# AI4Science-WestlakeU/wdno

Hardware: AMD Instinct MI355X
Metric: diffusion train steps/sec, 2D smoke U-Net (8 samples per GPU per step) (higher is better)
Workload: dtype f32

## Files before the change

include/wdno_hip.h:

```cpp
#ifndef WDNO_HIP_H
#define WDNO_HIP_H
#include <stdint.h>
#include <stddef.h>

#ifdef __cplusplus
extern "C" {
#endif

typedef void* wdno_stream_t;

enum { WDNO_OK = 0, WDNO_EINVAL = -1, WDNO_ELAUNCH = -2, WDNO_EUNSUPPORTED = -3, WDNO_EWORKSPACE = -4 };

#define WDNO_AMAX_SLOTS 64
#define WDNO_AMAX_STRIDE 16
#define WDNO_AMAX_FLOATS (WDNO_AMAX_SLOTS * WDNO_AMAX_STRIDE)
const char* wdno_strerror(int code);
int wdno_version(void);
const char* wdno_last_hip_error(void);
int wdno_set_debug(int mode);

typedef struct {
  int nd;
  int mode;
  int L;
  int n_img;
  int in_dims[3];
  int out_dims[3];
  int64_t cs_img, cs_band, cs0, cs1;
} wdno_dwt_desc;
size_t wdno_dwt_ws_bytes(const wdno_dwt_desc* d);
int wdno_dwt_fwd(const float* x, float* coef, const wdno_dwt_desc* d, const float* filters_host, void* ws, size_t ws_bytes, wdno_stream_t s);
int wdno_dwt_inv(const float* coef, float* x, const wdno_dwt_desc* d, const float* filters_host, void* ws, size_t ws_bytes, wdno_stream_t s);
int wdno_dwt_fwd_adjoint(const float* dcoef, float* dx, const wdno_dwt_desc* d, const float* filters_host, void* ws, size_t ws_bytes, wdno_stream_t s);
int wdno_dwt_inv_adjoint(const float* dx, float* dcoef, const wdno_dwt_desc* d, const float* filters_host, void* ws, size_t ws_bytes, wdno_stream_t s);
int wdno_dwt_fwd_packed(const float* x, float* state, const wdno_dwt_desc* d, const float* filters_host, int img_inner, int64_t cs_outer, int row_w,
                        const float* rescaler, wdno_stream_t s);
int wdno_upsample_coef(const float* in, float* out, int64_t outer, int a, int mid, int b, int c, int fa, int fb, int fc, wdno_stream_t s);
int wdno_pack_smoke_state(const float* coef, int64_t coef_sim_stride, const float* init_coef, int64_t init_sim_stride, const float* smokeout,
                          int64_t so_sim_stride, const int64_t* idx, const float* rescaler, float* state, int64_t B, int F, int nt, int nx,
                          int pad_t, int pad_x, wdno_stream_t s);
int wdno_pack_smoke_fields(const float* coef, int64_t coef_sim_stride, const float* rho0, int64_t rho0_sim_stride, const float* curve,
                           int64_t curve_sim_stride, const float* dec_lo_host, const float* dec_hi_host, int L, const float* rescaler,
                           float* state, int64_t B, int F, int nt, int nx, int pad_t, int pad_x, int H0, int W0, int T0, wdno_stream_t s);

int wdno_nc_to_cl(const float* src, float* dst, int64_t N, int C, int64_t S, int Cp, wdno_stream_t s);
int wdno_cl_to_nc(const float* src, float* dst, int64_t N, int C, int64_t S, int Cp, wdno_stream_t s);
int wdno_concat2_cl_planes(const float* a, int Ca, const float* b, int Cb, const float* rec_a, const float* rec_b, void* hi, void* lo,
                           float* scale_out, int64_t P, wdno_stream_t s);
int wdno_concat2_cl(const float* a, int Ca, const float* b, int Cb, float* out, int64_t P, wdno_stream_t s);
int wdno_concat2_cl_amax(const float* a, int Ca, const float* b, int Cb, float* out, float* amax_rec, int64_t P, wdno_stream_t s);
int wdno_split2_cl(const float* in, float* a, int Ca, float* b, int Cb, int64_t P, wdno_stream_t s);
int wdno_upsample2x_cl_fwd(const float* in, float* out, int64_t N, int H, int W, int C, wdno_stream_t s);
int wdno_upsample2x_cl_bwd(const float* dout, float* din, int64_t N, int H, int W, int C, wdno_stream_t s);

typedef struct {
  int N, D, H, W, C;
  int OD, OH, OW, K;
  int kd, kh, kw;
  int sd, sh, sw;
  int pd, ph, pw;
  int YD, YH, YW;
  int osd, osh, osw, ood, ooh, oow;
} wdno_conv_geom;
int wdno_conv_fwd(const float* x, const float* wp, const float* bias, const float* residual, float* y,
                  const wdno_conv_geom* g, wdno_stream_t s);
int wdno_amax(const float* x, int64_t n, float* amax_zeroed, wdno_stream_t s);
int wdno_amax_record(const float* x, int64_t n, float* rec_zeroed, wdno_stream_t s);
int wdno_split_f16(const float* x, const float* amax_rec, void* hi, void* lo, float* scale_out, int64_t rows, int C, int C8, wdno_stream_t s);
size_t wdno_split_colsum_ws_bytes(int64_t rows, int C8);
int wdno_split_f16_colsum(const float* x, const float* amax_rec, void* hi, void* lo, float* scale_out, float* colsum_out,
                          void* ws, size_t ws_bytes, int64_t rows, int C, int C8, wdno_stream_t s);
int wdno_pack_split_weight(const float* w, const float* amax, void* hi, void* lo, float* scale_out, int K, int C, int kd, int kh, int kw,
                           int A, int B, int mode, wdno_stream_t s);
typedef struct { const void* x; int64_t n; void* out; } wdno_amax_item;
typedef struct {
  const void* w; const void* amax; void* hi; void* lo; void* scale_out;
  int K, C, kd, kh, kw, A, B, mode;
} wdno_wsplit_item;
int wdno_amax_multi(const void* table, int n_items, int blocks_per_item, wdno_stream_t s);
int wdno_pack_split_weight_multi(const void* table, int n_items, int blocks_per_item, wdno_stream_t s);
int wdno_conv_fwd_f16x3(const void* xh, const void* xl, const float* sx, const void* wph, const void* wpl, const float* sw,
                        const float* bias, const float* residual, float* y, const wdno_conv_geom* g, wdno_stream_t s);
int wdno_conv_fwd_f16x3_amax(const void* xh, const void* xl, const float* sx, const void* wph, const void* wpl, const float* sw,
                             const float* bias, const float* residual, float* y, float* amax_rec, const wdno_conv_geom* g,
                             wdno_stream_t s);
typedef struct { int channels, d0, h0, w0; } wdno_zero_box;
int wdno_conv_fwd_f16x3_zbox(const void* xh, const void* xl, const float* sx, const void* wph, const void* wpl, const float* sw,
                             const float* bias, const float* residual, float* y, float* amax_rec, const wdno_conv_geom* g,
                             const wdno_zero_box* zb, wdno_stream_t s);
int wdno_conv_fwd_bf16_ex(const void* x16, const void* wp16, const float* bias, const float* residual, void* y, int y_bf16, float* amax_rec,
                          const wdno_conv_geom* g, const wdno_zero_box* zb, wdno_stream_t s);
int wdno_conv_fwd_f16x3_ws(const void* xh, const void* xl, const float* sx, const void* wph, const void* wpl, const float* sw,
                           const float* bias, const float* residual, float* y, float* amax_rec, const wdno_conv_geom* g,
                           void* ws, size_t ws_bytes, wdno_stream_t s);
size_t wdno_conv_fwd_split_ws_bytes(const wdno_conv_geom* g);
size_t wdno_conv_wgrad_f16x3_ws_bytes(const wdno_conv_geom* g);
int wdno_conv_pixel_table(void* table, const wdno_conv_geom* g, wdno_stream_t s);
int wdno_conv_wgrad_f16x3(const void* xh, const void* xl, const float* sx, const void* dyh, const void* dyl, const float* sdy,
                          const void* pixel_table, float* dwp, void* ws, size_t ws_bytes, const wdno_conv_geom* g, wdno_stream_t s);
int wdno_conv_wgrad_f16x3_param(const void* xh, const void* xl, const float* sx, const void* dyh, const void* dyl, const float* sdy,
                                const void* pixel_table, float* dw, int Kn, int Cn, void* ws, size_t ws_bytes,
                                const wdno_conv_geom* g, wdno_stream_t s);
#define WDNO_WGRAD_REDUCE_MAX 40
typedef struct wdno_wgrad_reduce_item {
  const float* ws; float* dw;
  int n, splits;
  int K8, C8, kw, ntap, Kn, Cn;
  int tiled;
  int reserved;
} wdno_wgrad_reduce_item;
int wdno_conv_wgrad_partials(const void* xh, const void* xl, const float* sx, const void* dyh, const void* dyl, const float* sdy,
                             const void* pixel_table, float* dw, int Kn, int Cn, void* ws, size_t ws_bytes,
                             const wdno_conv_geom* g, wdno_wgrad_reduce_item* item, wdno_stream_t s);
int wdno_wgrad_reduce_multi(const wdno_wgrad_reduce_item* items, int n_items, wdno_stream_t s);
size_t wdno_conv_wgrad_ws_bytes(const wdno_conv_geom* g);
int wdno_conv_wgrad(const float* x, const float* dy, float* dwp, void* ws, size_t ws_bytes,
                    const wdno_conv_geom* g, wdno_stream_t s);
#define WDNO_ROWS_SUM_MAX 64
typedef struct wdno_rows_sum_item {
  const void* part; float* out;
  int rows, stride, col0, ncols;
  int is_double, reserved;
} wdno_rows_sum_item;
int wdno_rows_sum_multi(const wdno_rows_sum_item* items, int n_items, wdno_stream_t s);
size_t wdno_colsum_ws_bytes(int64_t P, int C);
int wdno_colsum(const float* in, float* out, int64_t P, int C, void* ws, size_t ws_bytes, wdno_stream_t s);

int wdno_cast_bf16(const float* x, void* out16, int64_t rows, int C, int C8, wdno_stream_t s);
int wdno_cast_bf16_colsum(const float* x, void* out16, float* colsum_out, void* ws, size_t ws_bytes, int64_t rows, int C, int C8, wdno_stream_t s);
int wdno_conv_fwd_bf16(const void* x16, const void* wp16, const float* bias, const float* residual, float* y, float* amax_rec,
                       const wdno_conv_geom* g, wdno_stream_t s);
int wdno_conv_wgrad_bf16_param(const void* x16, const void* dy16, const void* pixel_table, float* dw, int Kn, int Cn, void* ws,
                               size_t ws_bytes, const wdno_conv_geom* g, wdno_stream_t s);

size_t wdno_groupnorm_ws_bytes(int64_t N, int64_t S, int C, int G);
size_t wdno_groupnorm_stats_floats(int64_t N, int C, int G);
int wdno_groupnorm_act_fwd(const float* x, const float* gamma, const float* beta, const float* ss, float* y,
                           float* stats, int64_t N, int64_t S, int C, int G, float eps, int silu,
                           void* ws, size_t ws_bytes, wdno_stream_t s);
int wdno_groupnorm_act_fwd_amax(const float* x, const float* gamma, const float* beta, const float* ss, float* y,
                                float* stats, float* amax_rec, int64_t N, int64_t S, int C, int G, float eps, int silu,
                                void* ws, size_t ws_bytes, wdno_stream_t s);
int wdno_groupnorm_act_bwd(const float* x, const float* dy, const float* gamma, const float* beta, const float* ss,
                           const float* stats, float* dx, float* dgb_partial, float* dss,
                           int64_t N, int64_t S, int C, int G, int silu, void* ws, size_t ws_bytes, wdno_stream_t s);
int wdno_groupnorm_act_bwd_amax(const float* x, const float* dy, const float* gamma, const float* beta, const float* ss,
                                const float* stats, float* dx, float* dgb_partial, float* dss, float* amax_rec,
                                int64_t N, int64_t S, int C, int G, int silu, void* ws, size_t ws_bytes, wdno_stream_t s);
size_t wdno_groupnorm_bwd_planes_ws_bytes(int64_t N, int64_t S, int C, int G);
size_t wdno_groupnorm_fwd_planes_ws_bytes(int64_t N, int64_t S, int C, int G);
int wdno_groupnorm_act_fwd_planes(const float* x, const float* gamma, const float* beta, const float* ss, void* y_hi, void* y_lo,
                                  float* y_scale, float* stats, float* bound_rec, int64_t N, int64_t S, int C, int G, float eps, int silu,
                                  void* ws, size_t ws_bytes, wdno_stream_t s);
int wdno_groupnorm_act_add_fwd_planes(const float* x, const float* gamma, const float* beta, const float* ss, const float* residual,
                                      const float* res_rec, float* y, void* y_hi, void* y_lo, float* y_scale, float* stats,
                                      float* bound_rec, float* y_amax_rec, int64_t N, int64_t S, int C, int G, float eps, int silu,
                                      void* ws, size_t ws_bytes, wdno_stream_t s);
int wdno_groupnorm_act_bwd_planes(const float* x, const float* dy, const float* gamma, const float* beta, const float* ss,
                                  const float* stats, void* dx_hi, void* dx_lo, float* dx_scale, float* dx_colsum,
                                  float* dgb_partial, float* dgb_sum, float* dss, float* bound_rec, int64_t N, int64_t S, int C, int G, int silu,
                                  void* ws, size_t ws_bytes, wdno_stream_t s);
int wdno_groupnorm_bwd_planes_tail(int64_t N, int64_t S, int C, int G, size_t* csp_offset, int* rows);
int wdno_groupnorm_act_fwd_amax_t(const void* x, int x_bf16, const float* gamma, const float* beta, const float* ss, float* y,
                                  float* stats, float* amax_rec, int64_t N, int64_t S, int C, int G, float eps, int silu,
                                  void* ws, size_t ws_bytes, wdno_stream_t s);
int wdno_groupnorm_act_fwd_planes_t(const void* x, int x_bf16, const float* gamma, const float* beta, const float* ss, void* y_hi, void* y_lo,
                                    float* y_scale, float* stats, float* bound_rec, int64_t N, int64_t S, int C, int G, float eps,
                                    int silu, void* ws, size_t ws_bytes, wdno_stream_t s);
int wdno_groupnorm_act_add_fwd_planes_t(const void* x, int x_bf16, const float* gamma, const float* beta, const float* ss, const float* residual,
                                        const float* res_rec, float* y, void* y_hi, void* y_lo, float* y_scale, float* stats,
                                        float* bound_rec, float* y_amax_rec, int64_t N, int64_t S, int C, int G, float eps, int silu,
                                        void* ws, size_t ws_bytes, wdno_stream_t s);
int wdno_groupnorm_act_bwd_planes_t(const void* x, int x_bf16, const void* dy, int dy_bf16, const float* gamma, const float* beta, const float* ss,
                                    const float* stats, void* dx_hi, void* dx_lo, float* dx_scale, float* dx_colsum,
                                    float* dgb_partial, float* dgb_sum, float* dss, float* bound_rec, int64_t N, int64_t S, int C, int G, int silu,
                                    void* ws, size_t ws_bytes, wdno_stream_t s);
int wdno_layernorm_fwd(const float* x, const float* g, float* y, int64_t P, int C, float eps, wdno_stream_t s);
int wdno_layernorm_fwd_amax(const float* x, const float* g, float* y, float* amax_rec, int64_t P, int C, float eps, wdno_stream_t s);
int wdno_layernorm_fwd_planes(const float* x, const float* g, void* y_hi, void* y_lo, float* y_scale, int64_t P, int C, float eps,
                              wdno_stream_t s);
size_t wdno_layernorm_bwd_ws_bytes(int64_t P, int C);
int wdno_layernorm_bwd(const float* x, const float* g, const float* dy, float* dx, float* dg, int64_t P, int C,
                       float eps, void* ws, size_t ws_bytes, wdno_stream_t s);
int wdno_layernorm_bwd_add(const float* x, const float* g, const float* dy, const float* add_to, float* dx, float* dg, int64_t P, int C,
                           float eps, void* ws, size_t ws_bytes, wdno_stream_t s);
int wdno_layernorm_bwd_add_amax(const float* x, const float* g, const float* dy, const float* add_to, float* dx, float* dg, float* amax_rec,
                                int64_t P, int C, float eps, void* ws, size_t ws_bytes, wdno_stream_t s);

typedef struct {
  int n_uo, n_ui, n_tok, heads;
  int64_t so, si, st;
} wdno_attn_desc;
int wdno_attn_fwd(const float* qkv, const float* rot_cos, const float* rot_sin, const float* bias, float* out,
                  const wdno_attn_desc* d, float scale, wdno_stream_t s);
size_t wdno_attn_bwd_ws_bytes(const wdno_attn_desc* d);
int wdno_attn_bwd(const float* qkv, const float* rot_cos, const float* rot_sin, const float* bias, const float* out,
                  const float* dout, float* dqkv, float* dbias, const wdno_attn_desc* d, float scale, void* ws, size_t ws_bytes,
                  wdno_stream_t s);
int wdno_attn_fwd_amax(const float* qkv, const float* rot_cos, const float* rot_sin, const float* bias, float* out, float* amax_rec,
                       const wdno_attn_desc* d, float scale, wdno_stream_t s);
int wdno_attn_bwd_amax(const float* qkv, const float* rot_cos, const float* rot_sin, const float* bias, const float* out,
                       const float* dout, float* dqkv, float* dbias, float* amax_rec, const wdno_attn_desc* d, float scale,
                       void* ws, size_t ws_bytes, wdno_stream_t s);
int wdno_attn_bwd_planes(const float* qkv, const float* rot_cos, const float* rot_sin, const float* bias, const float* out,
                         const float* dout, void* dqkv_hi, void* dqkv_lo, float* dqkv_scale, float* dbias,
                         const float* rec_qkv, const float* rec_dout, const wdno_attn_desc* d, float scale, void* ws, size_t ws_bytes,
                         wdno_stream_t s);
int wdno_attn_fwd_planes(const float* qkv, const float* rot_cos, const float* rot_sin, const float* bias, float* out, void* out_hi,
                         void* out_lo, float* out_scale, float* amax_rec, const float* rec_qkv, const wdno_attn_desc* d, float scale,
                         wdno_stream_t s);
size_t wdno_linattn_ws_bytes(int64_t units, int heads);
int wdno_linattn_fwd(const float* qkv, float* out, float* kstats , float* ctx ,
                     int64_t units, int n_tok, int heads, float scale, wdno_stream_t s);
int wdno_linattn_bwd(const float* qkv, const float* dout, const float* kstats, const float* ctx, float* dqkv,
                     void* ws, size_t ws_bytes, int64_t units, int n_tok, int heads, float scale, wdno_stream_t s);
int wdno_linattn_fwd_amax(const float* qkv, float* out, float* kstats, float* ctx, float* amax_rec, int64_t units, int n_tok, int heads,
                          float scale, wdno_stream_t s);
int wdno_linattn_bwd_amax(const float* qkv, const float* dout, const float* kstats, const float* ctx, float* dqkv, float* amax_rec,
                          void* ws, size_t ws_bytes, int64_t units, int n_tok, int heads, float scale, wdno_stream_t s);
int wdno_linattn_bwd_planes(const float* qkv, const float* dout, const float* kstats, const float* ctx, void* dqkv_hi, void* dqkv_lo,
                            float* dqkv_scale, const float* rec_qkv, const float* rec_dout, float* rec_dctx, void* ws, size_t ws_bytes,
                            int64_t units, int n_tok, int heads, float scale, wdno_stream_t s);
int wdno_linattn_fwd_planes(const float* qkv, void* out_hi, void* out_lo, float* out_scale, float* kstats, float* ctx,
                            const float* rec_qkv, int64_t units, int n_tok, int heads, float scale, wdno_stream_t s);

int wdno_tattn_fused_takes(int C, int n_tok, int heads);
int wdno_tattn_fused_fwd(const float* x, const float* gamma, float eps, const void* wq_hi, const void* wq_lo, const float* wq_scale,
                         const void* wo_hi, const void* wo_lo, const float* wo_scale, const float* rot_cos, const float* rot_sin,
                         const float* bias, float* y, float* amax_rec, float* qkv_out, float* rec_v,
                         int64_t n_batch, int n_tok, int64_t hw, int C, int heads, float scale, wdno_stream_t s);
size_t wdno_tattn_fused_bwd_ws_bytes(void);
int wdno_tattn_fused_bwd_grads(void);
int wdno_tattn_fused_bwd(const float* x, const float* dy, const float* gamma, float eps, const void* wq_hi, const void* wq_lo,
                         const float* wq_scale, const void* wo_hi, const void* wo_lo, const float* wo_scale, const float* rot_cos,
                         const float* rot_sin, const float* bias, const float* rec_dy, const float* rec_v, float* dx, float* amax_rec,
                         float* grads, void* ws, size_t ws_bytes,
                         int64_t n_batch, int n_tok, int64_t hw, int C, int heads, float scale, wdno_stream_t s);

int wdno_lattn_fused_takes(int C, int heads, int n_tok);
size_t wdno_lattn_fused_ws_bytes(int64_t units, int n_tok);
int wdno_lattn_fused_fwd(const float* x, const float* gamma, float eps, const void* wq_hi, const void* wq_lo, const float* wq_scale,
                         const void* wo_hi, const void* wo_lo, const float* wo_scale, const float* bias_out, float* y, float* amax_rec,
                         float* ctx_out, float* kstat_out, void* ws, size_t ws_bytes, int64_t units, int n_tok, int C, int heads, float scale,
                         wdno_stream_t s);

int wdno_lattn_fused_bwd_grads(void);
size_t wdno_lattn_fused_bwd_ws_bytes(int64_t units, int n_tok);
int wdno_lattn_fused_bwd(const float* x, const float* dy, const float* gamma, float eps, const void* wq_hi, const void* wq_lo,
                         const float* wq_scale, const void* wot_hi, const void* wot_lo, const float* wot_scale, const float* ctx,
                         const float* kstat, const float* rec_dy, float* dx, float* amax_rec, float* grads, void* ws, size_t ws_bytes,
                         int64_t units, int n_tok, int C, int heads, float scale, wdno_stream_t s);

int wdno_relpos_bias_fwd(const float* w, const int64_t* bucket, float* out, int n, int heads, wdno_stream_t s);
int wdno_relpos_bias_bwd(const float* dbias, const int64_t* bucket, float* dw, int n, int heads, int num_buckets, wdno_stream_t s);

int wdno_linear_rows_fwd(const float* x, int x_stride, const float* w, int w_stride, const float* bias, float* y, int P, int C, int K,
                         int Kp, wdno_stream_t s);
int wdno_linear_rows_wgrad(const float* x, int x_stride, const float* dy, int dy_stride, float* dw, float* db, int P, int C, int K,
                           wdno_stream_t s);

typedef struct wdno_linear_item {
  const void* w;
  const void* bias;
  int K, k_start;
} wdno_linear_item;
int wdno_linear_multi_fwd(const void* table, int n_items, int F, const float* x, float* y, int P, int C, wdno_stream_t s);
int wdno_linear_multi_wgrad(const void* table, int n_items, int F, const float* x, const float* dy, float* dw, float* db, int P, int C,
                            wdno_stream_t s);
size_t wdno_linear_multi_dgrad_ws_bytes(int F, int P, int C);
int wdno_linear_multi_dgrad(const void* table, int n_items, int F, const float* dy, float* dx, int P, int C, void* ws, size_t ws_bytes,
                            wdno_stream_t s);

int wdno_act_fwd(const float* x, float* y, int64_t n, int act, wdno_stream_t s);
int wdno_act_bwd(const float* x, const float* dy, float* dx, int64_t n, int act, wdno_stream_t s);
int wdno_add(const float* a, const float* b, float* out, int64_t n, wdno_stream_t s);
int wdno_add_amax(const float* a, const float* b, float* out, float* amax_rec, int64_t n, wdno_stream_t s);
int wdno_sinusoidal_emb(const int64_t* t, const float* freqs, float* out, int B, int dim, wdno_stream_t s);

typedef struct {
  int tree;
  int B, F, C, H, W;
  int cT, cH, cW;
  int cond_pad, cond_a, cond_b, cond_c, cond_low;
  int u_rows, uT_rows;
} wdno_cond_desc;
int wdno_q_sample_cond(const float* x0, const float* noise, const int64_t* t, const float* sqrt_ac, const float* sqrt_1mac,
                       float* x_out, float* target_out, const wdno_cond_desc* c, wdno_stream_t s);
int wdno_apply_cond(float* x, const float* src, const wdno_cond_desc* c, wdno_stream_t s);
int wdno_weighted_mse(const float* out, const float* target, const float* wc, const float* wb, float inv_count,
                      float* loss, float* grad, int64_t B, int64_t per_sample, int C, int64_t inner,
                      void* ws, size_t ws_bytes, wdno_stream_t s);
size_t wdno_weighted_mse_ws_bytes(int64_t n);
int wdno_weighted_mse_bwd(const float* out, const float* target, const float* wc, const float* wb, float inv_count,
                          const float* gscale, float* grad, int64_t B, int64_t per_sample, int C, int64_t inner, wdno_stream_t s);
int wdno_p_sample_update(const float* x, const float* eps, const float* noise, const int64_t* t,
                         const float* sqrt_recip_ac, const float* sqrt_recipm1_ac, const float* pm1, const float* pm2,
                         const float* plogvar, float* x_next, float* x_start, int64_t B, int64_t per_sample, int clamp, wdno_stream_t s);
int wdno_ddim_update(const float* x, const float* eps, const float* noise, const int64_t* t,
                     const float* sqrt_recip_ac, const float* sqrt_recipm1_ac, float sqrt_an, float c, float sigma,
                     float* x_next, float* x_start, int64_t B, int64_t per_sample, wdno_stream_t s);
int wdno_ddim_update_dev(const float* x, const float* eps, const float* noise, const int64_t* t,
                         const float* sqrt_recip_ac, const float* sqrt_recipm1_ac, const float* coef_dev,
                         float* x_next, float* x_start, int64_t B, int64_t per_sample, wdno_stream_t s);

size_t wdno_sumsq_ws_bytes(int64_t n);
int wdno_sumsq(const float* g, int64_t n, float* out, void* ws, size_t ws_bytes, wdno_stream_t s);
int wdno_adam_clip_step(float* p, const float* g, float* m, float* v, int64_t n, const float* sumsq, float max_norm,
                        float grad_scale, float lr, float beta1, float beta2, float eps, int step, wdno_stream_t s);
typedef struct { const void* src; void* dst; int64_t n; } wdno_copy_item;
int wdno_gather_items(const void* table, int n_items, int blocks_per_item, wdno_stream_t s);
int wdno_ema_update(float* ema, const float* p, int64_t n, float beta, wdno_stream_t s);

typedef struct {
  int N, s, nx0, nt_f, nxf;
  int steps, record_time, f_time, num_t, sub_s, out_cols;
  int waves, points;
  float c, d, dm, dt;
} wdno_burgers_desc;
int wdno_burgers_solve(const float* u0, const float* f, float* out, const wdno_burgers_desc* d, wdno_stream_t s);

typedef struct {
  int N, s, t;
  int steps, record_time, f_time, num_t;
  int st, sx, f_rows, cols;
  int waves, points, clamp;
  float c, d, dm, dt, alpha;
} wdno_burgers_generate_desc;
int wdno_burgers_generate(const float* u0, const float* ax, const float* tt, float* u_rec, float* f_rec,
                          const wdno_burgers_generate_desc* d, wdno_stream_t s);

typedef struct {
  int B, C, H, W;
  int sample_stride, chan_stride, row_stride;
  int h, w, n_t, n_x;
  int L, mode;
  int ntile, tw, lds_bytes;
  int num_timesteps;
  int condition_f, clip_x0;
  float wu, wf;
} wdno_burgers_guidance_desc;
int wdno_burgers_guidance(const float* x_t, const float* in, const int64_t* t, const float* c1, const float* c2, const float* s_table,
                          const float* rescaler, const float* target, float* out, const wdno_burgers_guidance_desc* d, const float* filt,
                          wdno_stream_t s);

typedef struct {
  int B, nt, nx, time_interval, space_interval;
  int num_t, max_iter, n_out, threads;
  float accuracy;
} wdno_smoke_solve_desc;
int wdno_smoke_solve(const float* init_density, const float* c1, const float* c2, const float* init_velocity, const float* fluid_ext,
                     const float* active_ext, const float* velocity_mask, const float* buckets, const int* frame_slot, float* density,
                     float* zero_density, float* velocity, double* ratio, float* ws, const wdno_smoke_solve_desc* d, wdno_stream_t s);

typedef struct {
  int B, scenelength, record_scale, stride;
  int max_iter, threads, noise_mode;
  float accuracy;
  unsigned long long seed;
} wdno_smoke_generate_desc;
int wdno_smoke_generate(const int* scene_i, const float* scene_v, const long long* scene_index, const double* noise,
                        const float* init_velocity, const float* fluid_ext, const float* active_ext, const float* velocity_mask,
                        const float* buckets, float* density, float* velocity, float* control, double* smoke, float* ws,
                        const wdno_smoke_generate_desc* d, wdno_stream_t s);
int wdno_smoke_noise(const long long* scene_index, const int* frame, const int* is_kick, const float* kick_v, int n,
                     unsigned long long seed, float* out, wdno_stream_t s);

#ifdef __cplusplus
}
#endif
#endif
```

wdno_amd/_lib.py:

```python
import contextlib
import ctypes as C
import os

import torch

HERE = os.path.dirname(os.path.abspath(__file__))
LIB_PATH = os.path.join(HERE, 'libwdno_hip.so')

P = C.c_void_p
I = C.c_int
L = C.c_int64
F = C.c_float
Z = C.c_size_t


class DwtDesc(C.Structure):
    _fields_ = [('nd', I), ('mode', I), ('L', I), ('n_img', I), ('in_dims', I * 3), ('out_dims', I * 3),
                ('cs_img', L), ('cs_band', L), ('cs0', L), ('cs1', L)]


class ConvGeom(C.Structure):
    _fields_ = [(k, I) for k in ('N', 'D', 'H', 'W', 'C', 'OD', 'OH', 'OW', 'K', 'kd', 'kh', 'kw', 'sd', 'sh', 'sw',
                                 'pd', 'ph', 'pw', 'YD', 'YH', 'YW', 'osd', 'osh', 'osw', 'ood', 'ooh', 'oow')]


class AttnDesc(C.Structure):
    _fields_ = [('n_uo', I), ('n_ui', I), ('n_tok', I), ('heads', I), ('so', L), ('si', L), ('st', L)]


class CondDesc(C.Structure):
    _fields_ = [(k, I) for k in ('tree', 'B', 'F', 'C', 'H', 'W', 'cT', 'cH', 'cW', 'cond_pad', 'cond_a', 'cond_b',
                                 'cond_c', 'cond_low', 'u_rows', 'uT_rows')]


class WgradReduceItem(C.Structure):
    _fields_ = [('ws', C.c_void_p), ('dw', C.c_void_p), ('n', I), ('splits', I), ('K8', I), ('C8', I), ('kw', I), ('ntap', I), ('Kn', I), ('Cn', I),
                ('tiled', I), ('reserved', I)]


class RowsSumItem(C.Structure):
    _fields_ = [('part', C.c_void_p), ('out', C.c_void_p), ('rows', I), ('stride', I), ('col0', I), ('ncols', I), ('is_double', I), ('reserved', I)]


class BurgersDesc(C.Structure):
    _fields_ = [(k, I) for k in ('N', 's', 'nx0', 'nt_f', 'nxf', 'steps', 'record_time', 'f_time', 'num_t', 'sub_s', 'out_cols', 'waves',
                                 'points')] + [(k, F) for k in ('c', 'd', 'dm', 'dt')]


class BurgersGenerateDesc(C.Structure):
    _fields_ = [(k, I) for k in ('N', 's', 't', 'steps', 'record_time', 'f_time', 'num_t', 'st', 'sx', 'f_rows', 'cols', 'waves', 'points',
                                 'clamp')] + [(k, F) for k in ('c', 'd', 'dm', 'dt', 'alpha')]


class BurgersGuidanceDesc(C.Structure):
    _fields_ = [(k, I) for k in ('B', 'C', 'H', 'W', 'sample_stride', 'chan_stride', 'row_stride', 'h', 'w', 'n_t', 'n_x', 'L', 'mode', 'ntile',
                                 'tw', 'lds_bytes', 'num_timesteps', 'condition_f', 'clip_x0')] + [(k, F) for k in ('wu', 'wf')]


class SmokeSolveDesc(C.Structure):
    _fields_ = [(k, I) for k in ('B', 'nt', 'nx', 'time_interval', 'space_interval', 'num_t', 'max_iter', 'n_out', 'threads')] + [('accuracy', F)]


class SmokeGenerateDesc(C.Structure):
    _fields_ = [(k, I) for k in ('B', 'scenelength', 'record_scale', 'stride', 'max_iter', 'threads', 'noise_mode')] + [('accuracy', F), ('seed', C.c_uint64)]


PD, PG, PA, PC = C.POINTER(DwtDesc), C.POINTER(ConvGeom), C.POINTER(AttnDesc), C.POINTER(CondDesc)
PF = C.POINTER(C.c_float)

PROTOTYPES = {
    'wdno_strerror': (C.c_char_p, [I]),
    'wdno_version': (I, []),
    'wdno_last_hip_error': (C.c_char_p, []),
    'wdno_set_debug': (I, [I]),
    'wdno_dwt_ws_bytes': (Z, [PD]),
    'wdno_dwt_fwd': (I, [P, P, PD, PF, P, Z, P]),
    'wdno_dwt_fwd_packed': (I, [P, P, PD, PF, I, L, I, P, P]),
    'wdno_dwt_inv': (I, [P, P, PD, PF, P, Z, P]),
    'wdno_dwt_fwd_adjoint': (I, [P, P, PD, PF, P, Z, P]),
    'wdno_dwt_inv_adjoint': (I, [P, P, PD, PF, P, Z, P]),
    'wdno_upsample_coef': (I, [P, P, L, I, I, I, I, I, I, I, P]),
    'wdno_pack_smoke_state': (I, [P, L, P, L, P, L, P, P, P, L, I, I, I, I, I, P]),
    'wdno_pack_smoke_fields': (I, [P, L, P, L, P, L, PF, PF, I, P, P, L, I, I, I, I, I, I, I, I, P]),
    'wdno_nc_to_cl': (I, [P, P, L, I, L, I, P]),
    'wdno_cl_to_nc': (I, [P, P, L, I, L, I, P]),
    'wdno_concat2_cl': (I, [P, I, P, I, P, L, P]),
    'wdno_concat2_cl_planes': (I, [P, I, P, I, P, P, P, P, P, L, P]),
    'wdno_concat2_cl_amax': (I, [P, I, P, I, P, P, L, P]),
    'wdno_split2_cl': (I, [P, P, I, P, I, L, P]),
    'wdno_upsample2x_cl_fwd': (I, [P, P, L, I, I, I, P]),
    'wdno_upsample2x_cl_bwd': (I, [P, P, L, I, I, I, P]),
    'wdno_conv_fwd': (I, [P, P, P, P, P, PG, P]),
    'wdno_amax': (I, [P, L, P, P]),
    'wdno_amax_record': (I, [P, L, P, P]),
    'wdno_split_f16': (I, [P, P, P, P, P, L, I, I, P]),
    'wdno_split_colsum_ws_bytes': (Z, [L, I]),
    'wdno_split_f16_colsum': (I, [P, P, P, P, P, P, P, Z, L, I, I, P]),
    'wdno_pack_split_weight': (I, [P, P, P, P, P, I, I, I, I, I, I, I, I, P]),
    'wdno_amax_multi': (I, [P, I, I, P]),
    'wdno_pack_split_weight_multi': (I, [P, I, I, P]),
    'wdno_conv_fwd_f16x3': (I, [P, P, P, P, P, P, P, P, P, PG, P]),
    'wdno_conv_fwd_f16x3_amax': (I, [P, P, P, P, P, P, P, P, P, P, PG, P]),
    'wdno_conv_fwd_f16x3_ws': (I, [P, P, P, P, P, P, P, P, P, P, PG, P, Z, P]),
    'wdno_conv_fwd_split_ws_bytes': (Z, [PG]),
    'wdno_conv_wgrad_f16x3_ws_bytes': (Z, [PG]),
    'wdno_conv_pixel_table': (I, [P, PG, P]),
    'wdno_conv_wgrad_f16x3': (I, [P, P, P, P, P, P, P, P, P, Z, PG, P]),
    'wdno_conv_wgrad_f16x3_param': (I, [P, P, P, P, P, P, P, P, I, I, P, Z, PG, P]),
    'wdno_conv_wgrad_partials': (I, [P, P, P, P, P, P, P, P, I, I, P, Z, PG, P, P]),
    'wdno_wgrad_reduce_multi': (I, [P, I, P]),
    'wdno_rows_sum_multi': (I, [P, I, P]),
    'wdno_cast_bf16': (I, [P, P, L, I, I, P]),
    'wdno_cast_bf16_colsum': (I, [P, P, P, P, Z, L, I, I, P]),
    'wdno_conv_fwd_bf16': (I, [P, P, P, P, P, P, PG, P]),
    'wdno_conv_fwd_f16x3_zbox': (I, [P, P, P, P, P, P, P, P, P, P, PG, P, P]),
    'wdno_conv_fwd_bf16_ex': (I, [P, P, P, P, P, I, P, PG, P, P]),
    'wdno_conv_wgrad_bf16_param': (I, [P, P, P, P, I, I, P, Z, PG, P]),
    'wdno_conv_wgrad_ws_bytes': (Z, [PG]),
    'wdno_conv_wgrad': (I, [P, P, P, P, Z, PG, P]),
    'wdno_colsum_ws_bytes': (Z, [L, I]),
    'wdno_colsum': (I, [P, P, L, I, P, Z, P]),
    'wdno_groupnorm_ws_bytes': (Z, [L, L, I, I]),
    'wdno_groupnorm_stats_floats': (Z, [L, I, I]),
    'wdno_groupnorm_act_fwd': (I, [P, P, P, P, P, P, L, L, I, I, F, I, P, Z, P]),
    'wdno_groupnorm_act_fwd_amax': (I, [P, P, P, P, P, P, P, L, L, I, I, F, I, P, Z, P]),
    'wdno_groupnorm_act_bwd': (I, [P, P, P, P, P, P, P, P, P, L, L, I, I, I, P, Z, P]),
    'wdno_groupnorm_act_bwd_amax': (I, [P, P, P, P, P, P, P, P, P, P, L, L, I, I, I, P, Z, P]),
    'wdno_groupnorm_bwd_planes_ws_bytes': (Z, [L, L, I, I]),
    'wdno_groupnorm_bwd_planes_tail': (I, [L, L, I, I, C.POINTER(Z), C.POINTER(I)]),
    'wdno_groupnorm_fwd_planes_ws_bytes': (Z, [L, L, I, I]),
    'wdno_groupnorm_act_fwd_planes': (I, [P, P, P, P, P, P, P, P, P, L, L, I, I, F, I, P, Z, P]),
    'wdno_groupnorm_act_add_fwd_planes': (I, [P, P, P, P, P, P, P, P, P, P, P, P, P, L, L, I, I, F, I, P, Z, P]),
    'wdno_layernorm_fwd_planes': (I, [P, P, P, P, P, L, I, F, P]),
    'wdno_groupnorm_act_bwd_planes': (I, [P, P, P, P, P, P, P, P, P, P, P, P, P, P, L, L, I, I, I, P, Z, P]),
    'wdno_groupnorm_act_fwd_amax_t': (I, [P, I, P, P, P, P, P, P, L, L, I, I, F, I, P, Z, P]),
    'wdno_groupnorm_act_fwd_planes_t': (I, [P, I, P, P, P, P, P, P, P, P, L, L, I, I, F, I, P, Z, P]),
    'wdno_groupnorm_act_add_fwd_planes_t': (I, [P, I, P, P, P, P, P, P, P, P, P, P, P, P, L, L, I, I, F, I, P, Z, P]),
    'wdno_groupnorm_act_bwd_planes_t': (I, [P, I, P, I, P, P, P, P, P, P, P, P, P, P, P, P, L, L, I, I, I, P, Z, P]),
    'wdno_layernorm_fwd': (I, [P, P, P, L, I, F, P]),
    'wdno_layernorm_fwd_amax': (I, [P, P, P, P, L, I, F, P]),
    'wdno_layernorm_bwd_ws_bytes': (Z, [L, I]),
    'wdno_layernorm_bwd': (I, [P, P, P, P, P, L, I, F, P, Z, P]),
    'wdno_layernorm_bwd_add': (I, [P, P, P, P, P, P, L, I, F, P, Z, P]),
    'wdno_layernorm_bwd_add_amax': (I, [P, P, P, P, P, P, P, L, I, F, P, Z, P]),
    'wdno_attn_fwd': (I, [P, P, P, P, P, PA, F, P]),
    'wdno_attn_bwd_ws_bytes': (Z, [PA]),
    'wdno_attn_bwd': (I, [P, P, P, P, P, P, P, P, PA, F, P, Z, P]),
    'wdno_attn_fwd_amax': (I, [P, P, P, P, P, P, PA, F, P]),
    'wdno_attn_bwd_amax': (I, [P, P, P, P, P, P, P, P, P, PA, F, P, Z, P]),
    'wdno_attn_fwd_planes': (I, [P, P, P, P, P, P, P, P, P, P, PA, F, P]),
    'wdno_linattn_fwd_planes': (I, [P, P, P, P, P, P, P, L, I, I, F, P]),
    'wdno_attn_bwd_planes': (I, [P, P, P, P, P, P, P, P, P, P, P, P, PA, F, P, Z, P]),
    'wdno_tattn_fused_takes': (I, [I, I, I]),
    'wdno_tattn_fused_fwd': (I, [P, P, F, P, P, P, P, P, P, P, P, P, P, P, P, P, L, I, L, I, I, F, P]),
    'wdno_lattn_fused_takes': (I, [I, I, I]),
    'wdno_lattn_fused_ws_bytes': (Z, [L, I]),
    'wdno_lattn_fused_fwd': (I, [P, P, F, P, P, P, P, P, P, P, P, P, P, P, P, Z, L, I, I, I, F, P]),
    'wdno_lattn_fused_bwd_grads': (I, []),
    'wdno_lattn_fused_bwd_ws_bytes': (Z, [L, I]),
    'wdno_lattn_fused_bwd': (I, [P, P, P, F, P, P, P, P, P, P, P, P, P, P, P, P, P, Z, L, I, I, I, F, P]),
    'wdno_tattn_fused_bwd_ws_bytes': (Z, []),
    'wdno_tattn_fused_bwd_grads': (I, []),
    'wdno_tattn_fused_bwd': (I, [P, P, P, F, P, P, P, P, P, P, P, P, P, P, P, P, P, P, P, Z, L, I, L, I, I, F, P]),
    'wdno_linattn_ws_bytes': (Z, [L, I]),
    'wdno_linattn_fwd': (I, [P, P, P, P, L, I, I, F, P]),
    'wdno_linattn_bwd': (I, [P, P, P, P, P, P, Z, L, I, I, F, P]),
    'wdno_linattn_fwd_amax': (I, [P, P, P, P, P, L, I, I, F, P]),
    'wdno_linattn_bwd_amax': (I, [P, P, P, P, P, P, P, Z, L, I, I, F, P]),
    'wdno_linattn_bwd_planes': (I, [P, P, P, P, P, P, P, P, P, P, P, Z, L, I, I, F, P]),
    'wdno_act_fwd': (I, [P, P, L, I, P]),
    'wdno_act_bwd': (I, [P, P, P, L, I, P]),
    'wdno_linear_rows_fwd': (I, [P, I, P, I, P, P, I, I, I, I, P]),
    'wdno_linear_rows_wgrad': (I, [P, I, P, I, P, P, I, I, I, P]),
    'wdno_linear_multi_fwd': (I, [P, I, I, P, P, I, I, P]),
    'wdno_linear_multi_wgrad': (I, [P, I, I, P, P, P, P, I, I, P]),
    'wdno_linear_multi_dgrad_ws_bytes': (Z, [I, I, I]),
    'wdno_linear_multi_dgrad': (I, [P, I, I, P, P, I, I, P, Z, P]),
    'wdno_add': (I, [P, P, P, L, P]),
    'wdno_add_amax': (I, [P, P, P, P, L, P]),
    'wdno_sinusoidal_emb': (I, [P, P, P, I, I, P]),
    'wdno_q_sample_cond': (I, [P, P, P, P, P, P, P, PC, P]),
    'wdno_apply_cond': (I, [P, P, PC, P]),
    'wdno_weighted_mse_ws_bytes': (Z, [L]),
    'wdno_weighted_mse': (I, [P, P, P, P, F, P, P, L, L, I, L, P, Z, P]),
    'wdno_weighted_mse_bwd': (I, [P, P, P, P, F, P, P, L, L, I, L, P]),
    'wdno_p_sample_update': (I, [P, P, P, P, P, P, P, P, P, P, P, L, L, I, P]),
    'wdno_ddim_update': (I, [P, P, P, P, P, P, F, F, F, P, P, L, L, P]),
    'wdno_ddim_update_dev': (I, [P, P, P, P, P, P, P, P, P, L, L, P]),
    'wdno_sumsq_ws_bytes': (Z, [L]),
    'wdno_sumsq': (I, [P, L, P, P, Z, P]),
    'wdno_adam_clip_step': (I, [P, P, P, P, L, P, F, F, F, F, F, F, I, P]),
    'wdno_ema_update': (I, [P, P, L, F, P]),
    'wdno_gather_items': (I, [P, I, I, P]),
    'wdno_relpos_bias_fwd': (I, [P, P, P, I, I, P]),
    'wdno_relpos_bias_bwd': (I, [P, P, P, I, I, I, P]),
    'wdno_burgers_solve': (I, [P, P, P, C.POINTER(BurgersDesc), P]),
    'wdno_burgers_generate': (I, [P, P, P, P, P, C.POINTER(BurgersGenerateDesc), P]),
    'wdno_burgers_guidance': (I, [P, P, P, P, P, P, P, P, P, C.POINTER(BurgersGuidanceDesc), PF, P]),
    'wdno_smoke_solve': (I, [P, P, P, P, P, P, P, P, P, P, P, P, P, P, C.POINTER(SmokeSolveDesc), P]),
    'wdno_smoke_generate': (I, [P, P, P, P, P, P, P, P, P, P, P, P, P, P, C.POINTER(SmokeGenerateDesc), P]),
    'wdno_smoke_noise': (I, [P, P, P, P, I, C.c_uint64, P, P]),
}

_lib = None


def load():
    global _lib
    if _lib is not None:
        return _lib
    if not os.path.exists(LIB_PATH):
        raise RuntimeError(f'{LIB_PATH} is missing: run `python -c "import __graft_entry__ as g; g.build()"` '
                           '(there is no CPU / eager fallback for the wdno_amd hot path)')
    lib = C.CDLL(LIB_PATH)
    for name, (res, args) in PROTOTYPES.items():
        fn = getattr(lib, name)
        fn.restype = res
        fn.argtypes = args
    _lib = lib
    if os.environ.get('WDNO_DEBUG'):
        try:
            check(lib.wdno_set_debug(int(os.environ['WDNO_DEBUG'])), f"WDNO_DEBUG={os.environ['WDNO_DEBUG']}")
        except RuntimeError:
            _lib = None
            raise
    return lib


def check(code, what):
    if code != 0:
        lib = load()
        msg = lib.wdno_strerror(code).decode()
        hip = lib.wdno_last_hip_error().decode() if code == -2 else ''
        raise RuntimeError(f'{what} failed: {msg} ({code}) {hip}')


@contextlib.contextmanager
def debug_mode(mode):
    lib = load()
    check(lib.wdno_set_debug(mode), f'wdno_set_debug({mode})')
    try:
        yield
    finally:
        lib.wdno_set_debug(0)
```

wdno_amd/csrc/common.h:

```cpp
#pragma once
#include <hip/hip_runtime.h>
#include <stdint.h>
#include "../../include/wdno_hip.h"

extern thread_local hipError_t wdno_tls_last_hip_error;

static inline int wdno_check_launch() {
  hipError_t e = hipGetLastError();
  if (e != hipSuccess) {
    wdno_tls_last_hip_error = e;
    return WDNO_ELAUNCH;
  }
  return WDNO_OK;
}

#define WDNO_REQUIRE(cond)            \
  do {                                \
    if (!(cond)) return WDNO_EINVAL;  \
  } while (0)

static inline hipStream_t as_stream(wdno_stream_t s) { return reinterpret_cast<hipStream_t>(s); }

int wdno_num_cus();

static inline int64_t cdiv64(int64_t a, int64_t b) { return (a + b - 1) / b; }
static inline int cdiv(int a, int b) { return (a + b - 1) / b; }

static inline int stream_grid(int64_t work_items, int block) {
  int64_t g = cdiv64(work_items, block);
  if (g > 2048) g = 2048;
  if (g < 1) g = 1;
  return (int)g;
}

#ifdef __HIPCC__
__device__ __forceinline__ float wave_sum(float v) {
#pragma unroll
  for (int o = 32; o > 0; o >>= 1) v += __shfl_xor(v, o, 64);
  return v;
}
__device__ __forceinline__ double wave_sum_d(double v) {
#pragma unroll
  for (int o = 32; o > 0; o >>= 1) v += __shfl_xor(v, o, 64);
  return v;
}
__device__ __forceinline__ float wave_max(float v) {
#pragma unroll
  for (int o = 32; o > 0; o >>= 1) v = fmaxf(v, __shfl_xor(v, o, 64));
  return v;
}
__device__ __forceinline__ void amax_record_emit(float m, float* __restrict__ rec, unsigned block_linear) {
  __shared__ float amax_red[4];
  m = wave_max(m);
  if ((threadIdx.x & 63) == 0) amax_red[(threadIdx.x >> 6) & 3] = m;
  __syncthreads();
  if (threadIdx.x == 0) {
    m = fmaxf(fmaxf(amax_red[0], amax_red[1]), fmaxf(amax_red[2], amax_red[3]));
    atomicMax(reinterpret_cast<unsigned*>(rec) + (block_linear & (WDNO_AMAX_SLOTS - 1)) * WDNO_AMAX_STRIDE, __float_as_uint(m));
  }
}
__device__ __forceinline__ void wave_amax_emit(float am, float* rec, int wave_linear) {
  am = wave_max(am);
  if ((threadIdx.x & 63) == 0)
    atomicMax(reinterpret_cast<unsigned*>(rec) + (wave_linear & (WDNO_AMAX_SLOTS - 1)) * WDNO_AMAX_STRIDE, __float_as_uint(am));
}
__device__ __forceinline__ float amax_record_read(const float* __restrict__ rec) {
  return wave_max(rec[(threadIdx.x & (WDNO_AMAX_SLOTS - 1)) * WDNO_AMAX_STRIDE]);
}
__device__ __forceinline__ unsigned short bf16_rne(float v) {
  unsigned u = __float_as_uint(v);
  if ((u & 0x7fffffffu) > 0x7f800000u) return (unsigned short)((u >> 16) | 0x40u);
  return (unsigned short)((u + 0x7fffu + ((u >> 16) & 1u)) >> 16);
}
__device__ __forceinline__ uint2 bf16x4_pack(float4 v) {
  return make_uint2((unsigned)bf16_rne(v.x) | ((unsigned)bf16_rne(v.y) << 16), (unsigned)bf16_rne(v.z) | ((unsigned)bf16_rne(v.w) << 16));
}
__device__ __forceinline__ void plane_pack(float v, float s, bool lp, _Float16& h, _Float16& l) {
  if (lp) { const unsigned short b = bf16_rne(v); h = __builtin_bit_cast(_Float16, b); l = (_Float16)0.f; return; }
  const float t = v * s;
  h = (_Float16)t;
  l = (_Float16)(t - (float)h);
}
__device__ __forceinline__ float scale_from_amax(float amax) {
  if (!(amax > 0.f) || !isfinite(amax)) return 1.0f;
  int e = ilogbf(amax);
  return ldexpf(1.0f, 14 - e);
}
__device__ __forceinline__ float amax4(float m, float4 v) {
  return fmaxf(fmaxf(m, fmaxf(fabsf(v.x), fabsf(v.y))), fmaxf(fabsf(v.z), fabsf(v.w)));
}
template <int W>
__device__ __forceinline__ float group_sum(float v) {
#pragma unroll
  for (int o = W / 2; o > 0; o >>= 1) v += __shfl_xor(v, o, 64);
  return v;
}
template <int W>
__device__ __forceinline__ float group_max(float v) {
#pragma unroll
  for (int o = W / 2; o > 0; o >>= 1) v = fmaxf(v, __shfl_xor(v, o, 64));
  return v;
}
#define PRS_GROUPS 32
#define PRS_THREADS (32 * PRS_GROUPS)
template <typename T>
__device__ __forceinline__ void partial_rows_sum_body(const T* __restrict__ part, float* __restrict__ out, int nb, int C, int bx, int stride = 0) {
  __shared__ double red[PRS_GROUPS][33];
  const int tx = threadIdx.x & 31, ty = threadIdx.x >> 5;
  const int c = bx * 32 + tx;
  if (stride == 0) stride = C;
  double acc = 0.0;
  if (c < C) {
    double a0 = 0.0, a1 = 0.0, a2 = 0.0, a3 = 0.0;
    int b = ty;
    for (; b + 3 * PRS_GROUPS < nb; b += 4 * PRS_GROUPS) {
      a0 += (double)part[(int64_t)b * stride + c];
      a1 += (double)part[(int64_t)(b + PRS_GROUPS) * stride + c];
      a2 += (double)part[(int64_t)(b + 2 * PRS_GROUPS) * stride + c];
      a3 += (double)part[(int64_t)(b + 3 * PRS_GROUPS) * stride + c];
    }
    for (; b < nb; b += PRS_GROUPS) a0 += (double)part[(int64_t)b * stride + c];
    acc = (a0 + a1) + (a2 + a3);
  }
  red[ty][tx] = acc;
  __syncthreads();
  if (ty == 0 && c < C) {
    double a[4] = {0.0, 0.0, 0.0, 0.0};
#pragma unroll
    for (int g = 0; g < PRS_GROUPS; ++g) a[g & 3] += red[g][tx];
    out[c] = (float)((a[0] + a[1]) + (a[2] + a[3]));
  }
}
template <typename T>
__global__ __launch_bounds__(PRS_THREADS) void partial_rows_sum_kernel(const T* __restrict__ part, float* __restrict__ out, int nb, int C) {
  partial_rows_sum_body<T>(part, out, nb, C, (int)blockIdx.x);
}

__device__ __forceinline__ float silu_f(float z) { return z / (1.0f + expf(-z)); }
__device__ __forceinline__ float silu_grad_f(float z) {
  float sg = 1.0f / (1.0f + expf(-z));
  return sg * (1.0f + z * (1.0f - sg));
}
#endif
```

wdno_amd/csrc/norm.hip:

```cpp
#include "common.h"
#include <type_traits>

#define GN_MAXC 1024

struct gn_bf16 {};
template <typename T> struct gn_ld;
template <> struct gn_ld<float> {
  static __device__ __forceinline__ float4 ld4(const void* p, int64_t e) { return *reinterpret_cast<const float4*>(static_cast<const float*>(p) + e); }
};
template <> struct gn_ld<gn_bf16> {
  static __device__ __forceinline__ float4 ld4(const void* p, int64_t e) {
    const uint2 u = *reinterpret_cast<const uint2*>(static_cast<const unsigned short*>(p) + e);
    return make_float4(__uint_as_float(u.x << 16), __uint_as_float(u.x & 0xffff0000u), __uint_as_float(u.y << 16), __uint_as_float(u.y & 0xffff0000u));
  }
};
template <typename T> __device__ __forceinline__ void gn_ld8(const void* p, int64_t e, float (&v)[8]) {
  const float4 a = gn_ld<T>::ld4(p, e), b = gn_ld<T>::ld4(p, e + 4);
  v[0] = a.x; v[1] = a.y; v[2] = a.z; v[3] = a.w; v[4] = b.x; v[5] = b.y; v[6] = b.z; v[7] = b.w;
}

static inline int pow2ceil(int v) { int p = 1; while (p < v) p <<= 1; return p; }
static inline int gn_chunks(int64_t S, int64_t N, int C) {
  int64_t c = cdiv64(S, 64);
  if (c > 64) c = 64;
  if (c < 1) c = 1;
  int txp = pow2ceil(C >> 2);
  if (txp > 256) txp = 256;
  const int nty = 256 / (txp < 1 ? 1 : txp);
  const int64_t cap = N > 0 && 512 / N > 64 ? 512 / N : 64;
  while (c < cap && N * c < 256 && S / (2 * c) >= 4 * nty) c *= 2;
  return (int)c;
}

template <int MODE, typename XT = float, typename DT = float>
__global__ __launch_bounds__(256) void gn_partial_kernel(const void* __restrict__ x, const void* __restrict__ dy,
                                                          const float* __restrict__ cb , const float* __restrict__ gb ,
                                                          double* __restrict__ part, int64_t S, int C, int cg, int G, int txp,
                                                          int64_t rows_per_chunk, int silu, float* __restrict__ mx = nullptr) {
  __shared__ double red[256 * 8];
  __shared__ float redm[8];
  float m0[4] = {0.f, 0.f, 0.f, 0.f}, m1[4] = {0.f, 0.f, 0.f, 0.f};
  const int n = blockIdx.y, chunk = blockIdx.x, nchunk = gridDim.x;
  const int C4 = C >> 2;
  const int tx = threadIdx.x & (txp - 1), ty = threadIdx.x / txp, nty = 256 / txp;
  const int64_t r0 = (int64_t)chunk * rows_per_chunk;
  int64_t r1 = r0 + rows_per_chunk;
  if (r1 > S) r1 = S;
  double s0[4] = {0, 0, 0, 0}, s1[4] = {0, 0, 0, 0};
  if (tx < C4) {
    float ca[4], cbb[4], mean[4], rstd[4];
    if (MODE == 1) {
#pragma unroll
      for (int j = 0; j < 4; ++j) {
        int c = tx * 4 + j;
        ca[j] = cb[((int64_t)n * C + c) * 4 + 0];
        cbb[j] = cb[((int64_t)n * C + c) * 4 + 1];
        int g = c / cg;
        mean[j] = gb[((int64_t)n * G + g) * 4 + 0];
        rstd[j] = gb[((int64_t)n * G + g) * 4 + 1];
      }
    }
    const int64_t e0 = ((int64_t)n * S) * C + tx * 4;
    constexpr int RIF = std::is_same<XT, gn_bf16>::value ? 8 : 4;
    for (int64_t rb = r0 + ty; rb < r1; rb += RIF * nty) {
      float4 vv[RIF], dd[RIF];
#pragma unroll
      for (int u = 0; u < RIF; ++u) {
        const int64_t r = rb + u * nty;
        const bool ok = r < r1;
        vv[u] = ok ? gn_ld<XT>::ld4(x, e0 + r * C) : make_float4(0.f, 0.f, 0.f, 0.f);
        if (MODE == 1) dd[u] = ok ? gn_ld<DT>::ld4(dy, e0 + r * C) : make_float4(0.f, 0.f, 0.f, 0.f);
      }
#pragma unroll
      for (int u = 0; u < RIF; ++u) {
        if (rb + u * nty >= r1) break;
        const float4 v = vv[u];
        float xv[4] = {v.x, v.y, v.z, v.w};
        if (MODE == 0) {
#pragma unroll
          for (int j = 0; j < 4; ++j) { s0[j] += (double)xv[j]; s1[j] += (double)xv[j] * (double)xv[j]; m0[j] = fmaxf(m0[j], fabsf(xv[j])); }
        } else {
          const float4 d = dd[u];
          float dv[4] = {d.x, d.y, d.z, d.w};
#pragma unroll
          for (int j = 0; j < 4; ++j) {
            float dz = dv[j];
            if (silu) dz *= silu_grad_f(ca[j] * xv[j] + cbb[j]);
            float xh = (xv[j] - mean[j]) * rstd[j];
            s0[j] += (double)dz;
            s1[j] += (double)dz * (double)xh;
            m0[j] = fmaxf(m0[j], fabsf(dz)); m1[j] = fmaxf(m1[j], fabsf(xh));
          }
        }
      }
    }
  }
#pragma unroll
  for (int j = 0; j < 4; ++j) { red[(ty * txp + tx) * 8 + j] = s0[j]; red[(ty * txp + tx) * 8 + 4 + j] = s1[j]; }
  __syncthreads();
  if (ty == 0 && tx < C4) {
    for (int t = 1; t < nty; ++t)
#pragma unroll
      for (int j = 0; j < 4; ++j) { s0[j] += red[(t * txp + tx) * 8 + j]; s1[j] += red[(t * txp + tx) * 8 + 4 + j]; }
    double* o = part + (((int64_t)n * nchunk + chunk) * C + tx * 4) * 2;
#pragma unroll
    for (int j = 0; j < 4; ++j) { o[j * 2] = s0[j]; o[j * 2 + 1] = s1[j]; }
  }
  if (mx) {
    float a = fmaxf(fmaxf(m0[0], m0[1]), fmaxf(m0[2], m0[3])), b = fmaxf(fmaxf(m1[0], m1[1]), fmaxf(m1[2], m1[3]));
    a = wave_max(a); b = wave_max(b);
    if ((threadIdx.x & 63) == 0) { redm[(threadIdx.x >> 6) * 2] = a; redm[(threadIdx.x >> 6) * 2 + 1] = b; }
    __syncthreads();
    if (threadIdx.x == 0) {
      float* o = mx + ((int64_t)n * nchunk + chunk) * 2;
      o[0] = fmaxf(fmaxf(redm[0], redm[2]), fmaxf(redm[4], redm[6]));
      o[1] = fmaxf(fmaxf(redm[1], redm[3]), fmaxf(redm[5], redm[7]));
    }
  }
}

__device__ __forceinline__ void gn_chunk_totals(const double* __restrict__ part, int n, int nchunk, int Call, double* sa, double* sb, int cb0 = 0, int cn = -1) {
  const int C = cn < 0 ? Call : cn;
  part += cb0 * 2;
  const int nsub = C <= 128 ? 256 / C : 1;
  for (int idx = threadIdx.x; idx < C * nsub; idx += 256) {
    const int q = idx / C, c = idx - q * C;
    const int k1 = (q + 1) * nchunk / nsub;
    int k = q * nchunk / nsub;
    double a0 = 0, b0 = 0, a1 = 0, b1 = 0;
    for (; k + 7 < k1; k += 8) {
      const double* q0 = part + (((int64_t)n * nchunk + k) * Call + c) * 2;
      double va[8], vb[8];
#pragma unroll
      for (int u = 0; u < 8; ++u) { va[u] = q0[(int64_t)u * Call * 2]; vb[u] = q0[(int64_t)u * Call * 2 + 1]; }
#pragma unroll
      for (int u = 0; u < 8; u += 2) { a0 += va[u]; b0 += vb[u]; a1 += va[u + 1]; b1 += vb[u + 1]; }
    }
    for (; k + 1 < k1; k += 2) {
      const double* q0 = part + (((int64_t)n * nchunk + k) * Call + c) * 2;
      const double* q1 = q0 + (int64_t)Call * 2;
      a0 += q0[0]; b0 += q0[1]; a1 += q1[0]; b1 += q1[1];
    }
    if (k < k1) {
      const double* q0 = part + (((int64_t)n * nchunk + k) * Call + c) * 2;
      a0 += q0[0]; b0 += q0[1];
    }
    sa[idx] = a0 + a1; sb[idx] = b0 + b1;
  }
  __syncthreads();
  if (nsub > 1) {
    const int c = threadIdx.x;
    double a = 0, b = 0;
    if (c < C)
      for (int q = 0; q < nsub; ++q) { a += sa[q * C + c]; b += sb[q * C + c]; }
    __syncthreads();
    if (c < C) { sa[c] = a; sb[c] = b; }
    __syncthreads();
  }
}

__global__ __launch_bounds__(256) void gn_finalize_kernel(const double* __restrict__ part, const float* __restrict__ stats_in,
                                                           const float* __restrict__ gamma, const float* __restrict__ beta,
                                                           const float* __restrict__ ss, float* __restrict__ stats_out,
                                                           float* __restrict__ cb, float* __restrict__ gb, int64_t S, int C, int G,
                                                           int nchunk, float eps, const float* __restrict__ mx = nullptr,
                                                           float* __restrict__ bound_rec = nullptr) {
  __shared__ double chs[GN_MAXC], chq[GN_MAXC];
  __shared__ float gmean[GN_MAXC], grstd[GN_MAXC];
  const int n = blockIdx.x, cg = C / G;
  const int gps = (G + (int)gridDim.y - 1) / (int)gridDim.y, gs0 = (int)blockIdx.y * gps, gs1 = min(G, gs0 + gps);
  if (gs0 >= gs1) return;
  const int cs0 = gs0 * cg, csn = (gs1 - gs0) * cg;
  gamma += cs0; beta += cs0;
  if (ss) ss += cs0;
  cb += (int64_t)cs0 * 4; gb += (int64_t)gs0 * 4;
  if (stats_out) stats_out += (int64_t)gs0 * 2;
  if (stats_in) stats_in += (int64_t)gs0 * 2;
  const int Call = C, Gall = G;
  C = csn; G = gs1 - gs0;
  if (part) {
    gn_chunk_totals(part, n, nchunk, Call, chs, chq, cs0, csn);
    if (cg > 64) {
      __shared__ double ra[256], rb[256];
      for (int g = 0; g < G; ++g) {
        double a = 0, b = 0;
        for (int c = g * cg + threadIdx.x; c < (g + 1) * cg; c += 256) { a += chs[c]; b += chq[c]; }
        ra[threadIdx.x] = a; rb[threadIdx.x] = b;
        __syncthreads();
        for (int o = 128; o > 0; o >>= 1) {
          if (threadIdx.x < o) { ra[threadIdx.x] += ra[threadIdx.x + o]; rb[threadIdx.x] += rb[threadIdx.x + o]; }
          __syncthreads();
        }
        if (threadIdx.x == 0) { chs[g * cg] = ra[0]; chq[g * cg] = rb[0]; }
        __syncthreads();
      }
    }
    for (int g = threadIdx.x; g < G; g += 256) {
      double a = 0, b = 0;
      if (cg > 64) { a = chs[g * cg]; b = chq[g * cg]; }
      else for (int c = g * cg; c < (g + 1) * cg; ++c) { a += chs[c]; b += chq[c]; }
      double m = (double)cg * (double)S;
      double mean = a / m;
      double var = b / m - mean * mean;
      if (var < 0) var = 0;
      float rstd = (float)(1.0 / sqrt(var + (double)eps));
      gmean[g] = (float)mean; grstd[g] = rstd;
      stats_out[((int64_t)n * Gall + g) * 2 + 0] = (float)mean;
      stats_out[((int64_t)n * Gall + g) * 2 + 1] = rstd;
    }
  } else {
    for (int g = threadIdx.x; g < G; g += 256) {
      gmean[g] = stats_in[((int64_t)n * Gall + g) * 2 + 0];
      grstd[g] = stats_in[((int64_t)n * Gall + g) * 2 + 1];
    }
  }
  __syncthreads();
  for (int g = threadIdx.x; g < G; g += 256) {
    float* o = gb + ((int64_t)n * Gall + g) * 4;
    o[0] = gmean[g]; o[1] = grstd[g]; o[2] = 0.f; o[3] = 0.f;
  }
  float ma = 0.f, mb = 0.f;
  for (int c = threadIdx.x; c < C; c += 256) {
    int g = c / cg;
    float sc1 = ss ? ss[(int64_t)n * 2 * Call + c] + 1.0f : 1.0f;
    float sh = ss ? ss[(int64_t)n * 2 * Call + Call + c] : 0.0f;
    float k1 = grstd[g] * gamma[c];
    float a = k1 * sc1;
    float b = (beta[c] - gmean[g] * k1) * sc1 + sh;
    float* o = cb + ((int64_t)n * Call + c) * 4;
    o[0] = a; o[1] = b; o[2] = a; o[3] = 0.f;
    ma = fmaxf(ma, fabsf(a)); mb = fmaxf(mb, fabsf(b));
  }
  if (bound_rec) {
    float mxx = 0.f;
    for (int k = threadIdx.x; k < nchunk; k += 256) mxx = fmaxf(mxx, mx[((int64_t)n * nchunk + k) * 2]);
    __shared__ float bm[3][4];
    float v[3] = {wave_max(ma), wave_max(mb), wave_max(mxx)};
    if ((threadIdx.x & 63) == 0)
      for (int q = 0; q < 3; ++q) bm[q][threadIdx.x >> 6] = v[q];
    __syncthreads();
    if (threadIdx.x == 0) {
      float t[3];
      for (int q = 0; q < 3; ++q) t[q] = fmaxf(fmaxf(bm[q][0], bm[q][1]), fmaxf(bm[q][2], bm[q][3]));
      atomicMax(reinterpret_cast<unsigned*>(bound_rec) + (n & (WDNO_AMAX_SLOTS - 1)) * WDNO_AMAX_STRIDE, __float_as_uint(t[0] * t[2] + t[1]));
    }
  }
}

template <typename XT = float>
__global__ __launch_bounds__(256) void gn_apply_kernel(const void* __restrict__ x, const float* __restrict__ cb, float* __restrict__ y,
                                                        int64_t S, int C, int silu, float* __restrict__ amax_rec) {
  const int n = blockIdx.y;
  const int C4 = C >> 2;
  const int64_t total4 = S * C4;
  const int64_t xe = (int64_t)n * S * C;
  float4* yp = reinterpret_cast<float4*>(y + (int64_t)n * S * C);
  const float4* cbp = reinterpret_cast<const float4*>(cb + (int64_t)n * C * 4);
  const int64_t stride = (int64_t)gridDim.x * 256;
  float am = 0.f;
  for (int64_t i = (int64_t)blockIdx.x * 256 + threadIdx.x; i < total4; i += stride) {
    int c4 = (int)(i % C4);
    float4 v = gn_ld<XT>::ld4(x, xe + i * 4);
    float4 k0 = cbp[c4 * 4 + 0], k1 = cbp[c4 * 4 + 1], k2 = cbp[c4 * 4 + 2], k3 = cbp[c4 * 4 + 3];
    float4 o;
    o.x = k0.x * v.x + k0.y; o.y = k1.x * v.y + k1.y; o.z = k2.x * v.z + k2.y; o.w = k3.x * v.w + k3.y;
    if (silu) { o.x = silu_f(o.x); o.y = silu_f(o.y); o.z = silu_f(o.z); o.w = silu_f(o.w); }
    yp[i] = o;
    am = amax4(am, o);
  }
  if (amax_rec) amax_record_emit(am, amax_rec, blockIdx.y * gridDim.x + blockIdx.x);
}

__global__ __launch_bounds__(256) void gn_bwd_finalize_kernel(const double* __restrict__ part, const float* __restrict__ gamma,
                                                               const float* __restrict__ beta, const float* __restrict__ ss,
                                                               float* __restrict__ gb, float* __restrict__ dgb, float* __restrict__ dss,
                                                               int64_t S, int C, int G, int nchunk, const float* __restrict__ cb = nullptr,
                                                               const float* __restrict__ mx = nullptr, float* __restrict__ bound_rec = nullptr) {
  __shared__ double chA[GN_MAXC], chB[GN_MAXC];
  const int n = blockIdx.x, cg = C / G;
  const int gps = (G + (int)gridDim.y - 1) / (int)gridDim.y, gs0 = (int)blockIdx.y * gps, gs1 = min(G, gs0 + gps);
  if (gs0 >= gs1) return;
  const int cs0 = gs0 * cg, csn = (gs1 - gs0) * cg;
  gamma += cs0; beta += cs0;
  if (ss) ss += cs0;
  if (dss) dss += cs0;
  dgb += cs0; gb += (int64_t)gs0 * 4;
  if (cb) cb += (int64_t)cs0 * 4;
  const int Call = C, Gall = G;
  C = csn; G = gs1 - gs0;
  gn_chunk_totals(part, n, nchunk, Call, chA, chB, cs0, csn);
  for (int c = threadIdx.x; c < C; c += 256) {
    const double a = chA[c], b = chB[c];
    float sc1 = ss ? ss[(int64_t)n * 2 * Call + c] + 1.0f : 1.0f;
    if (dss) {
      dss[(int64_t)n * 2 * Call + c] = (float)((double)gamma[c] * b + (double)beta[c] * a);
      dss[(int64_t)n * 2 * Call + Call + c] = (float)a;
    }
    dgb[((int64_t)n * 2 + 0) * Call + c] = (float)((double)sc1 * b);
    dgb[((int64_t)n * 2 + 1) * Call + c] = (float)((double)sc1 * a);
    double w = (double)gamma[c] * (double)sc1;
    chA[c] = w * a; chB[c] = w * b;
  }
  __syncthreads();
  if (cg > 64) {
    __shared__ double ra[256], rb[256];
    for (int g = 0; g < G; ++g) {
      double a = 0, b = 0;
      for (int c = g * cg + threadIdx.x; c < (g + 1) * cg; c += 256) { a += chA[c]; b += chB[c]; }
      ra[threadIdx.x] = a; rb[threadIdx.x] = b;
      __syncthreads();
      for (int o = 128; o > 0; o >>= 1) {
        if (threadIdx.x < o) { ra[threadIdx.x] += ra[threadIdx.x + o]; rb[threadIdx.x] += rb[threadIdx.x + o]; }
        __syncthreads();
      }
      if (threadIdx.x == 0) { chA[g * cg] = ra[0]; chB[g * cg] = rb[0]; }
      __syncthreads();
    }
  }
  for (int g = threadIdx.x; g < G; g += 256) {
    double a = 0, b = 0;
    if (cg > 64) { a = chA[g * cg]; b = chB[g * cg]; }
    else for (int c = g * cg; c < (g + 1) * cg; ++c) { a += chA[c]; b += chB[c]; }
    double m = (double)cg * (double)S;
    float* o = gb + ((int64_t)n * Gall + g) * 4;
    float rstd = o[1];
    o[2] = (float)(a / m) * rstd;
    o[3] = (float)(b / m) * rstd;
  }
  if (bound_rec) {
    __syncthreads();
    float mdz = 0.f, mxh = 0.f, mk = 0.f, mz = 0.f, mw = 0.f;
    for (int k = threadIdx.x; k < nchunk; k += 256) {
      mdz = fmaxf(mdz, mx[((int64_t)n * nchunk + k) * 2]); mxh = fmaxf(mxh, mx[((int64_t)n * nchunk + k) * 2 + 1]);
    }
    for (int c = threadIdx.x; c < C; c += 256) mk = fmaxf(mk, fabsf(cb[((int64_t)n * Call + c) * 4 + 2]));
    for (int g = threadIdx.x; g < G; g += 256) {
      mz = fmaxf(mz, fabsf(gb[((int64_t)n * Gall + g) * 4 + 2])); mw = fmaxf(mw, fabsf(gb[((int64_t)n * Gall + g) * 4 + 3]));
    }
    __shared__ float bm[5][4];
    float v[5] = {wave_max(mdz), wave_max(mxh), wave_max(mk), wave_max(mz), wave_max(mw)};
    if ((threadIdx.x & 63) == 0)
      for (int q = 0; q < 5; ++q) bm[q][threadIdx.x >> 6] = v[q];
    __syncthreads();
    if (threadIdx.x == 0) {
      float t[5];
      for (int q = 0; q < 5; ++q) t[q] = fmaxf(fmaxf(bm[q][0], bm[q][1]), fmaxf(bm[q][2], bm[q][3]));
      const float bound = t[2] * t[0] + t[3] + t[1] * t[4];
      atomicMax(reinterpret_cast<unsigned*>(bound_rec) + (n & (WDNO_AMAX_SLOTS - 1)) * WDNO_AMAX_STRIDE, __float_as_uint(bound));
    }
  }
}

__global__ __launch_bounds__(256) void gn_bwd_apply_kernel(const float* __restrict__ x, const float* __restrict__ dy,
                                                            const float* __restrict__ cb, const float* __restrict__ gb,
                                                            float* __restrict__ dx, int64_t S, int C, int cg, int G, int silu,
                                                            float* __restrict__ amax_rec) {
  const int n = blockIdx.y;
  const int C4 = C >> 2;
  const int64_t total4 = S * C4;
  const float4* xp = reinterpret_cast<const float4*>(x + (int64_t)n * S * C);
  const float4* dp = reinterpret_cast<const float4*>(dy + (int64_t)n * S * C);
  float4* op = reinterpret_cast<float4*>(dx + (int64_t)n * S * C);
  const float4* cbp = reinterpret_cast<const float4*>(cb + (int64_t)n * C * 4);
  const float4* gbp = reinterpret_cast<const float4*>(gb + (int64_t)n * G * 4);
  const int64_t stride = (int64_t)gridDim.x * 256;
  float am = 0.f;
  for (int64_t i = (int64_t)blockIdx.x * 256 + threadIdx.x; i < total4; i += stride) {
    int c4 = (int)(i % C4);
    float4 v = xp[i], d = dp[i];
    float xv[4] = {v.x, v.y, v.z, v.w}, dv[4] = {d.x, d.y, d.z, d.w}, o[4];
#pragma unroll
    for (int j = 0; j < 4; ++j) {
      int c = c4 * 4 + j;
      float4 k = cbp[c];
      float4 gq = gbp[c / cg];
      float dz = dv[j];
      if (silu) dz *= silu_grad_f(k.x * xv[j] + k.y);
      float xh = (xv[j] - gq.x) * gq.y;
      o[j] = k.z * dz - gq.z - xh * gq.w;
    }
    op[i] = make_float4(o[0], o[1], o[2], o[3]);
    am = fmaxf(fmaxf(am, fmaxf(fabsf(o[0]), fabsf(o[1]))), fmaxf(fabsf(o[2]), fabsf(o[3])));
  }
  if (amax_rec) amax_record_emit(am, amax_rec, blockIdx.y * gridDim.x + blockIdx.x);
}

typedef _Float16 gn_half8 __attribute__((ext_vector_type(8)));
template <typename XT = float>
__global__ __launch_bounds__(256) void gn_apply_planes_kernel(const void* __restrict__ x, const float* __restrict__ cb,
                                                               _Float16* __restrict__ hi, _Float16* __restrict__ lo,
                                                               float* __restrict__ scale_out, const float* __restrict__ rec,
                                                               int64_t S, int C, int silu) {
  const int n = blockIdx.y;
  const int C8 = C >> 3;
  const int64_t total8 = S * C8;
  const bool single = lo == nullptr;
  const float s = single ? 1.0f : scale_from_amax(amax_record_read(rec));
  if (!single && blockIdx.x == 0 && blockIdx.y == 0 && threadIdx.x == 0) scale_out[0] = s;
  const int64_t xe = (int64_t)n * S * C;
  _Float16* hp = hi + (int64_t)n * S * C;
  _Float16* lp = single ? nullptr : lo + (int64_t)n * S * C;
  const float4* cbp = reinterpret_cast<const float4*>(cb + (int64_t)n * C * 4);
  const int64_t stride = (int64_t)gridDim.x * 256;
  const int c0 = (int)(((int64_t)blockIdx.x * 256 + threadIdx.x) % C8) * 8;
  float ka[8], kb[8];
#pragma unroll
  for (int j = 0; j < 8; ++j) { const float4 k = cbp[c0 + j]; ka[j] = k.x; kb[j] = k.y; }
  for (int64_t i = (int64_t)blockIdx.x * 256 + threadIdx.x; i < total8; i += stride) {
    float xv[8];
    gn_ld8<XT>(x, xe + i * 8, xv);
    gn_half8 h, l;
#pragma unroll
    for (int j = 0; j < 8; ++j) {
      float o = ka[j] * xv[j] + kb[j];
      if (silu) o = silu_f(o);
      _Float16 th, tl;
      plane_pack(o, s, single, th, tl);
      h[j] = th; l[j] = tl;
    }
    *reinterpret_cast<gn_half8*>(hp + i * 8) = h;
    if (!single) *reinterpret_cast<gn_half8*>(lp + i * 8) = l;
  }
}

template <typename XT = float>
__global__ __launch_bounds__(256) void gn_apply_add_planes_kernel(const void* __restrict__ x, const float* __restrict__ cb,
                                                                   const float* __restrict__ res, float* __restrict__ y,
                                                                   _Float16* __restrict__ hi, _Float16* __restrict__ lo,
                                                                   float* __restrict__ scale_out, const float* __restrict__ rec,
                                                                   const float* __restrict__ rec_res, float* __restrict__ amax_out,
                                                                   int64_t S, int C, int silu) {
  const int n = blockIdx.y;
  const int C8 = C >> 3;
  const int64_t total8 = S * C8;
  const bool planes = hi != nullptr;
  const bool single = lo == nullptr;
  const float s = single ? 1.0f : scale_from_amax(amax_record_read(rec) + amax_record_read(rec_res));
  if (!single && blockIdx.x == 0 && blockIdx.y == 0 && threadIdx.x == 0) scale_out[0] = s;
  const int64_t xe = (int64_t)n * S * C;
  const float* rp = res + (int64_t)n * S * C;
  float* yp = y + (int64_t)n * S * C;
  _Float16* hp = planes ? hi + (int64_t)n * S * C : nullptr;
  _Float16* lp = single ? nullptr : lo + (int64_t)n * S * C;
  const float4* cbp = reinterpret_cast<const float4*>(cb + (int64_t)n * C * 4);
  const int64_t stride = (int64_t)gridDim.x * 256;
  const int c0 = (int)(((int64_t)blockIdx.x * 256 + threadIdx.x) % C8) * 8;
  float ka[8], kb[8];
#pragma unroll
  for (int j = 0; j < 8; ++j) { const float4 k = cbp[c0 + j]; ka[j] = k.x; kb[j] = k.y; }
  float am = 0.f;
  for (int64_t i = (int64_t)blockIdx.x * 256 + threadIdx.x; i < total8; i += stride) {
    float xv[8];
    gn_ld8<XT>(x, xe + i * 8, xv);
    const float4 r0 = *reinterpret_cast<const float4*>(rp + i * 8), r1 = *reinterpret_cast<const float4*>(rp + i * 8 + 4);
    const float rv[8] = {r0.x, r0.y, r0.z, r0.w, r1.x, r1.y, r1.z, r1.w};
    float ov[8];
    gn_half8 h, l;
#pragma unroll
    for (int j = 0; j < 8; ++j) {
      float o = ka[j] * xv[j] + kb[j];
      if (silu) o = silu_f(o);
      o += rv[j];
      ov[j] = o;
      am = fmaxf(am, fabsf(o));
      _Float16 th, tl;
      plane_pack(o, s, single, th, tl);
      h[j] = th; l[j] = tl;
    }
    *reinterpret_cast<float4*>(yp + i * 8) = make_float4(ov[0], ov[1], ov[2], ov[3]);
    *reinterpret_cast<float4*>(yp + i * 8 + 4) = make_float4(ov[4], ov[5], ov[6], ov[7]);
    if (planes) *reinterpret_cast<gn_half8*>(hp + i * 8) = h;
    if (planes && !single) *reinterpret_cast<gn_half8*>(lp + i * 8) = l;
  }
  if (amax_out) amax_record_emit(am, amax_out, blockIdx.y * gridDim.x + blockIdx.x);
}

template <typename XT = float, typename DT = float>
__global__ __launch_bounds__(256) void gn_bwd_apply_planes_kernel(const void* __restrict__ x, const void* __restrict__ dy,
                                                                   const float* __restrict__ cb, const float* __restrict__ gb,
                                                                   _Float16* __restrict__ hi, _Float16* __restrict__ lo,
                                                                   float* __restrict__ scale_out, const float* __restrict__ rec,
                                                                   double* __restrict__ csp, int64_t S, int C, int cg, int G, int silu) {
  __shared__ double red[256][9];
  const int n = blockIdx.y;
  const int C8 = C >> 3;
  const int64_t total8 = S * C8;
  const bool single = lo == nullptr;
  const float s = single ? 1.0f : scale_from_amax(amax_record_read(rec));
  if (!single && blockIdx.x == 0 && blockIdx.y == 0 && threadIdx.x == 0) scale_out[0] = s;
  const int64_t xe = (int64_t)n * S * C;
  _Float16* hp = hi + (int64_t)n * S * C;
  _Float16* lp = single ? nullptr : lo + (int64_t)n * S * C;
  const float4* cbp = reinterpret_cast<const float4*>(cb + (int64_t)n * C * 4);
  const float4* gbp = reinterpret_cast<const float4*>(gb + (int64_t)n * G * 4);
  const int64_t stride = (int64_t)gridDim.x * 256;
  const int c0 = (int)(((int64_t)blockIdx.x * 256 + threadIdx.x) % C8) * 8;
  float4 kk[8], gq[8];
#pragma unroll
  for (int j = 0; j < 8; ++j) { kk[j] = cbp[c0 + j]; gq[j] = gbp[(c0 + j) / cg]; }
  double acc[8] = {0, 0, 0, 0, 0, 0, 0, 0};
  for (int64_t i = (int64_t)blockIdx.x * 256 + threadIdx.x; i < total8; i += stride) {
    float xv[8], dv[8];
    gn_ld8<XT>(x, xe + i * 8, xv);
    gn_ld8<DT>(dy, xe + i * 8, dv);
    gn_half8 h, l;
#pragma unroll
    for (int j = 0; j < 8; ++j) {
      float dz = dv[j];
      if (silu) dz *= silu_grad_f(kk[j].x * xv[j] + kk[j].y);
      const float xh = (xv[j] - gq[j].x) * gq[j].y;
      const float o = kk[j].z * dz - gq[j].z - xh * gq[j].w;
      acc[j] += (double)o;
      _Float16 th, tl;
      plane_pack(o, s, single, th, tl);
      h[j] = th; l[j] = tl;
    }
    *reinterpret_cast<gn_half8*>(hp + i * 8) = h;
    if (!single) *reinterpret_cast<gn_half8*>(lp + i * 8) = l;
  }
#pragma unroll
  for (int j = 0; j < 8; ++j) red[threadIdx.x][j] = acc[j];
  __syncthreads();
  if (threadIdx.x < C8) {
    for (int t = threadIdx.x + C8; t < 256; t += C8)
#pragma unroll
      for (int j = 0; j < 8; ++j) acc[j] += red[t][j];
    double* o = csp + ((int64_t)n * gridDim.x + blockIdx.x) * C + c0;
#pragma unroll
    for (int j = 0; j < 8; ++j) o[j] = acc[j];
  }
}

extern "C" size_t wdno_groupnorm_ws_bytes(int64_t N, int64_t S, int C, int G) {
  size_t part = (size_t)N * gn_chunks(S, N, C) * C * 2 * sizeof(double);
  return part + (size_t)N * C * 4 * sizeof(float) + (size_t)N * G * 4 * sizeof(float) + 64;
}
extern "C" size_t wdno_groupnorm_stats_floats(int64_t N, int C, int G) { return (size_t)N * G * 2 + (size_t)N * C * 4 + (size_t)N * G * 4; }
static inline float* gn_cb(float* stats, int64_t N, int G) { return stats + (size_t)N * G * 2; }
static inline float* gn_gb(float* stats, int64_t N, int C, int G) { return stats + (size_t)N * G * 2 + (size_t)N * C * 4; }
static inline unsigned gn_slices(int C, int G) { return C / G > 64 ? 1u : (unsigned)(G < 32 ? G : 32); }
static int gn_check(int64_t N, int64_t S, int C, int G) {
  if (N <= 0 || S <= 0 || C <= 0 || G <= 0 || N > 65535) return WDNO_EINVAL;
  if ((C & 3) || C > GN_MAXC || (C % G) != 0) return WDNO_EUNSUPPORTED;
  return WDNO_OK;
}
#define GN_PARTIAL0(XB, ...) do { if (XB) gn_partial_kernel<0, gn_bf16><<<__VA_ARGS__; else gn_partial_kernel<0, float><<<__VA_ARGS__; } while (0)
extern "C" int wdno_groupnorm_act_fwd_amax_t(const void* x, int x_bf16, const float* gamma, const float* beta, const float* ss, float* y,
                                      float* stats, float* amax_rec, int64_t N, int64_t S, int C, int G, float eps, int silu,
                                      void* ws, size_t ws_bytes, wdno_stream_t s) {
  int rc = gn_check(N, S, C, G);
  if (rc) return rc;
  if (ws_bytes < wdno_groupnorm_ws_bytes(N, S, C, G)) return WDNO_EWORKSPACE;
  const int nchunk = gn_chunks(S, N, C);
  double* part = (double*)ws;
  float* cb = gn_cb(stats, N, G);
  float* gb = gn_gb(stats, N, C, G);
  const int txp = pow2ceil(C / 4);
  const int64_t rpc = cdiv64(S, nchunk);
  hipStream_t st = as_stream(s);
  GN_PARTIAL0(x_bf16, dim3(nchunk, (unsigned)N), 256, 0, st>>>(x, nullptr, nullptr, nullptr, part, S, C, C / G, G, txp, rpc, 0));
  gn_finalize_kernel<<<dim3((unsigned)N, gn_slices(C, G)), 256, 0, st>>>(part, nullptr, gamma, beta, ss, stats, cb, gb, S, C, G, nchunk, eps);
  int gx = stream_grid(S * (C / 4), 256);
  if (gx > 512) gx = 512;
  if (x_bf16) gn_apply_kernel<gn_bf16><<<dim3(gx, (unsigned)N), 256, 0, st>>>(x, cb, y, S, C, silu, amax_rec);
  else gn_apply_kernel<float><<<dim3(gx, (unsigned)N), 256, 0, st>>>(x, cb, y, S, C, silu, amax_rec);
  return wdno_check_launch();
}
extern "C" int wdno_groupnorm_act_fwd_amax(const float* x, const float* gamma, const float* beta, const float* ss, float* y,
                                      float* stats, float* amax_rec, int64_t N, int64_t S, int C, int G, float eps, int silu,
                                      void* ws, size_t ws_bytes, wdno_stream_t s) {
  return wdno_groupnorm_act_fwd_amax_t(x, 0, gamma, beta, ss, y, stats, amax_rec, N, S, C, G, eps, silu, ws, ws_bytes, s);
}
extern "C" int wdno_groupnorm_act_fwd(const float* x, const float* gamma, const float* beta, const float* ss, float* y,
                                      float* stats, int64_t N, int64_t S, int C, int G, float eps, int silu,
                                      void* ws, size_t ws_bytes, wdno_stream_t s) {
  return wdno_groupnorm_act_fwd_amax(x, gamma, beta, ss, y, stats, nullptr, N, S, C, G, eps, silu, ws, ws_bytes, s);
}
extern "C" int wdno_groupnorm_act_bwd_amax(const float* x, const float* dy, const float* gamma, const float* beta, const float* ss,
                                      const float* stats, float* dx, float* dgb_partial, float* dss, float* amax_rec,
                                      int64_t N, int64_t S, int C, int G, int silu, void* ws, size_t ws_bytes, wdno_stream_t s) {
  int rc = gn_check(N, S, C, G);
  if (rc) return rc;
  if (ws_bytes < wdno_groupnorm_ws_bytes(N, S, C, G)) return WDNO_EWORKSPACE;
  const int nchunk = gn_chunks(S, N, C);
  double* part = (double*)ws;
  const float* cb = gn_cb(const_cast<float*>(stats), N, G);
  float* gb = gn_gb(const_cast<float*>(stats), N, C, G);
  const int txp = pow2ceil(C / 4);
  const int64_t rpc = cdiv64(S, nchunk);
  hipStream_t st = as_stream(s);
  gn_partial_kernel<1><<<dim3(nchunk, (unsigned)N), 256, 0, st>>>(x, dy, cb, gb, part, S, C, C / G, G, txp, rpc, silu);
  gn_bwd_finalize_kernel<<<dim3((unsigned)N, gn_slices(C, G)), 256, 0, st>>>(part, gamma, beta, ss, gb, dgb_partial, dss, S, C, G, nchunk);
  int gx = stream_grid(S * (C / 4), 256);
  if (gx > 512) gx = 512;
  gn_bwd_apply_kernel<<<dim3(gx, (unsigned)N), 256, 0, st>>>(x, dy, cb, gb, dx, S, C, C / G, G, silu, amax_rec);
  return wdno_check_launch();
}
extern "C" int wdno_groupnorm_act_bwd(const float* x, const float* dy, const float* gamma, const float* beta, const float* ss,
                                      const float* stats, float* dx, float* dgb_partial, float* dss,
                                      int64_t N, int64_t S, int C, int G, int silu, void* ws, size_t ws_bytes, wdno_stream_t s) {
  return wdno_groupnorm_act_bwd_amax(x, dy, gamma, beta, ss, stats, dx, dgb_partial, dss, nullptr, N, S, C, G, silu, ws, ws_bytes, s);
}


extern "C" size_t wdno_groupnorm_fwd_planes_ws_bytes(int64_t N, int64_t S, int C, int G) {
  return wdno_groupnorm_ws_bytes(N, S, C, G) + (size_t)N * gn_chunks(S, N, C) * 2 * sizeof(float) + 128;
}
extern "C" int wdno_groupnorm_act_fwd_planes_t(const void* x, int x_bf16, const float* gamma, const float* beta, const float* ss, void* y_hi, void* y_lo,
                                             float* y_scale, float* stats, float* bound_rec, int64_t N, int64_t S, int C, int G, float eps,
                                             int silu, void* ws, size_t ws_bytes, wdno_stream_t s) {
  int rc = gn_check(N, S, C, G);
  if (rc) return rc;
  const int C8 = C / 8;
  if ((C & 7) || C8 > 256 || (C8 & (C8 - 1))) return WDNO_EUNSUPPORTED;
  if (ws_bytes < wdno_groupnorm_fwd_planes_ws_bytes(N, S, C, G)) return WDNO_EWORKSPACE;
  const int nchunk = gn_chunks(S, N, C);
  double* part = (double*)ws;
  float* cb = gn_cb(stats, N, G);
  float* gb = gn_gb(stats, N, C, G);
  float* mx = (float*)((char*)ws + ((wdno_groupnorm_ws_bytes(N, S, C, G) + 63) & ~(size_t)63));
  const int txp = pow2ceil(C / 4);
  const int64_t rpc = cdiv64(S, nchunk);
  hipStream_t st = as_stream(s);
  GN_PARTIAL0(x_bf16, dim3(nchunk, (unsigned)N), 256, 0, st>>>(x, nullptr, nullptr, nullptr, part, S, C, C / G, G, txp, rpc, 0, y_lo ? mx : nullptr));
  gn_finalize_kernel<<<dim3((unsigned)N, gn_slices(C, G)), 256, 0, st>>>(part, nullptr, gamma, beta, ss, stats, cb, gb, S, C, G, nchunk, eps, mx, y_lo ? bound_rec : nullptr);
  int gx = stream_grid(S * (C / 8), 256);
  if (gx > 512) gx = 512;
  if (x_bf16) gn_apply_planes_kernel<gn_bf16><<<dim3(gx, (unsigned)N), 256, 0, st>>>(x, cb, (_Float16*)y_hi, (_Float16*)y_lo, y_scale, bound_rec, S, C, silu);
  else gn_apply_planes_kernel<float><<<dim3(gx, (unsigned)N), 256, 0, st>>>(x, cb, (_Float16*)y_hi, (_Float16*)y_lo, y_scale, bound_rec, S, C, silu);
  return wdno_check_launch();
}
extern "C" int wdno_groupnorm_act_fwd_planes(const float* x, const float* gamma, const float* beta, const float* ss, void* y_hi, void* y_lo,
                                             float* y_scale, float* stats, float* bound_rec, int64_t N, int64_t S, int C, int G, float eps,
                                             int silu, void* ws, size_t ws_bytes, wdno_stream_t s) {
  return wdno_groupnorm_act_fwd_planes_t(x, 0, gamma, beta, ss, y_hi, y_lo, y_scale, stats, bound_rec, N, S, C, G, eps, silu, ws, ws_bytes, s);
}

extern "C" int wdno_groupnorm_act_add_fwd_planes_t(const void* x, int x_bf16, const float* gamma, const float* beta, const float* ss, const float* residual,
                                                 const float* res_rec, float* y, void* y_hi, void* y_lo, float* y_scale, float* stats,
                                                 float* bound_rec, float* y_amax_rec, int64_t N, int64_t S, int C, int G, float eps, int silu,
                                                 void* ws, size_t ws_bytes, wdno_stream_t s) {
  int rc = gn_check(N, S, C, G);
  if (rc) return rc;
  const int C8 = C / 8;
  if ((C & 7) || C8 > 256 || (C8 & (C8 - 1))) return WDNO_EUNSUPPORTED;
  if (!residual || !y || (y_lo && (!y_hi || !res_rec || !bound_rec || !y_scale))) return WDNO_EINVAL;
  if (ws_bytes < wdno_groupnorm_fwd_planes_ws_bytes(N, S, C, G)) return WDNO_EWORKSPACE;
  const int nchunk = gn_chunks(S, N, C);
  double* part = (double*)ws;
  float* cb = gn_cb(stats, N, G);
  float* gb = gn_gb(stats, N, C, G);
  float* mx = (float*)((char*)ws + ((wdno_groupnorm_ws_bytes(N, S, C, G) + 63) & ~(size_t)63));
  const int txp = pow2ceil(C / 4);
  const int64_t rpc = cdiv64(S, nchunk);
  hipStream_t st = as_stream(s);
  GN_PARTIAL0(x_bf16, dim3(nchunk, (unsigned)N), 256, 0, st>>>(x, nullptr, nullptr, nullptr, part, S, C, C / G, G, txp, rpc, 0, y_lo ? mx : nullptr));
  gn_finalize_kernel<<<dim3((unsigned)N, gn_slices(C, G)), 256, 0, st>>>(part, nullptr, gamma, beta, ss, stats, cb, gb, S, C, G, nchunk, eps, mx, y_lo ? bound_rec : nullptr);
  int gx = stream_grid(S * (C / 8), 256);
  if (gx > 512) gx = 512;
  if (x_bf16) gn_apply_add_planes_kernel<gn_bf16><<<dim3(gx, (unsigned)N), 256, 0, st>>>(x, cb, residual, y, (_Float16*)y_hi, (_Float16*)y_lo, y_scale, bound_rec,
                                                                                       res_rec, y_amax_rec, S, C, silu);
  else gn_apply_add_planes_kernel<float><<<dim3(gx, (unsigned)N), 256, 0, st>>>(x, cb, residual, y, (_Float16*)y_hi, (_Float16*)y_lo, y_scale, bound_rec, res_rec,
                                                                           y_amax_rec, S, C, silu);
  return wdno_check_launch();
}
extern "C" int wdno_groupnorm_act_add_fwd_planes(const float* x, const float* gamma, const float* beta, const float* ss, const float* residual,
                                                 const float* res_rec, float* y, void* y_hi, void* y_lo, float* y_scale, float* stats,
                                                 float* bound_rec, float* y_amax_rec, int64_t N, int64_t S, int C, int G, float eps, int silu,
                                                 void* ws, size_t ws_bytes, wdno_stream_t s) {
  return wdno_groupnorm_act_add_fwd_planes_t(x, 0, gamma, beta, ss, residual, res_rec, y, y_hi, y_lo, y_scale, stats, bound_rec, y_amax_rec, N, S, C, G, eps, silu,
                                             ws, ws_bytes, s);
}

__global__ __launch_bounds__(PRS_THREADS) void gn_bwd_tail_kernel(const double* __restrict__ csp, float* __restrict__ dx_colsum, int nb, int C, int nbx,
                                                                     const float* __restrict__ dgb, float* __restrict__ dgb_sum, int N) {
  if ((int)blockIdx.x < nbx) {
    partial_rows_sum_body<double>(csp, dx_colsum, nb, C, (int)blockIdx.x);
    return;
  }
  partial_rows_sum_body<float>(dgb, dgb_sum, N, 2 * C, (int)blockIdx.x - nbx);
}

static inline int gn_planes_grid(int64_t N, int64_t S, int C) {
  int gx = stream_grid(S * (C / 8), 256);
  int cap = (int)(2048 / N);
  if (cap < 2) cap = 2;
  if (cap > 128) cap = 128;
  if (gx > cap) gx = cap;
  return gx;
}
extern "C" size_t wdno_groupnorm_bwd_planes_ws_bytes(int64_t N, int64_t S, int C, int G) {
  return wdno_groupnorm_ws_bytes(N, S, C, G) + (size_t)N * gn_chunks(S, N, C) * 2 * sizeof(float) + (size_t)N * 128 * C * sizeof(double) + 64;
}
extern "C" int wdno_groupnorm_bwd_planes_tail(int64_t N, int64_t S, int C, int G, size_t* csp_offset, int* rows) {
  int rc = gn_check(N, S, C, G);
  if (rc) return rc;
  WDNO_REQUIRE(csp_offset && rows);
  *csp_offset = (wdno_groupnorm_ws_bytes(N, S, C, G) + 63) & ~(size_t)63;
  *rows = (int)N * gn_planes_grid(N, S, C);
  return WDNO_OK;
}
extern "C" int wdno_groupnorm_act_bwd_planes_t(const void* x, int x_bf16, const void* dy, int dy_bf16, const float* gamma, const float* beta, const float* ss,
                                             const float* stats, void* dx_hi, void* dx_lo, float* dx_scale, float* dx_colsum,
                                             float* dgb_partial, float* dgb_sum, float* dss, float* bound_rec, int64_t N, int64_t S, int C, int G, int silu,
                                             void* ws, size_t ws_bytes, wdno_stream_t s) {
  int rc = gn_check(N, S, C, G);
  if (rc) return rc;
  const int C8 = C / 8;
  if ((C & 7) || C8 > 256 || (C8 & (C8 - 1))) return WDNO_EUNSUPPORTED;
  if (ws_bytes < wdno_groupnorm_bwd_planes_ws_bytes(N, S, C, G)) return WDNO_EWORKSPACE;
  const int nchunk = gn_chunks(S, N, C);
  double* part = (double*)ws;
  const float* cb = gn_cb(const_cast<float*>(stats), N, G);
  float* gb = gn_gb(const_cast<float*>(stats), N, C, G);
  char* tail = (char*)ws + ((wdno_groupnorm_ws_bytes(N, S, C, G) + 63) & ~(size_t)63);
  double* csp = (double*)tail;
  float* mx = (float*)(csp + (size_t)N * 128 * C);
  const int txp = pow2ceil(C / 4);
  const int64_t rpc = cdiv64(S, nchunk);
  hipStream_t st = as_stream(s);
#define GN_BWD_TYPES(KERNEL, ...) do { \
    if (x_bf16 && dy_bf16) KERNEL(gn_bf16, gn_bf16, __VA_ARGS__); else if (x_bf16) KERNEL(gn_bf16, float, __VA_ARGS__); \
    else if (dy_bf16) KERNEL(float, gn_bf16, __VA_ARGS__); else KERNEL(float, float, __VA_ARGS__); } while (0)
#define GN_K_PARTIAL1(XT, DT, ...) gn_partial_kernel<1, XT, DT><<<dim3(nchunk, (unsigned)N), 256, 0, st>>>(__VA_ARGS__)
#define GN_K_BWD_APPLY(XT, DT, ...) gn_bwd_apply_planes_kernel<XT, DT><<<dim3(gx, (unsigned)N), 256, 0, st>>>(__VA_ARGS__)
  GN_BWD_TYPES(GN_K_PARTIAL1, x, dy, cb, gb, part, S, C, C / G, G, txp, rpc, silu, dx_lo ? mx : nullptr);
  gn_bwd_finalize_kernel<<<dim3((unsigned)N, gn_slices(C, G)), 256, 0, st>>>(part, gamma, beta, ss, gb, dgb_partial, dss, S, C, G, nchunk, cb, mx, dx_lo ? bound_rec : nullptr);
  const int gx = gn_planes_grid(N, S, C);
  GN_BWD_TYPES(GN_K_BWD_APPLY, x, dy, cb, gb, (_Float16*)dx_hi, (_Float16*)dx_lo, dx_scale, bound_rec, csp, S, C, C / G, G, silu);
  const int nbx = dx_colsum ? cdiv(C, 32) : 0, nby = dgb_sum ? cdiv(2 * C, 32) : 0;
  if (nbx + nby) gn_bwd_tail_kernel<<<nbx + nby, PRS_THREADS, 0, st>>>(csp, dx_colsum, (int)N * gx, C, nbx, dgb_partial, dgb_sum, (int)N);
  return wdno_check_launch();
}

extern "C" int wdno_groupnorm_act_bwd_planes(const float* x, const float* dy, const float* gamma, const float* beta, const float* ss,
                                             const float* stats, void* dx_hi, void* dx_lo, float* dx_scale, float* dx_colsum,
                                             float* dgb_partial, float* dgb_sum, float* dss, float* bound_rec, int64_t N, int64_t S, int C, int G, int silu,
                                             void* ws, size_t ws_bytes, wdno_stream_t s) {
  return wdno_groupnorm_act_bwd_planes_t(x, 0, dy, 0, gamma, beta, ss, stats, dx_hi, dx_lo, dx_scale, dx_colsum, dgb_partial, dgb_sum, dss, bound_rec, N, S, C, G,
                                         silu, ws, ws_bytes, s);
}

template <int TPR, int VPL, bool BWD>
__global__ __launch_bounds__(256) void layernorm_kernel(const float* __restrict__ x, const float* __restrict__ g,
                                                         const float* __restrict__ dy, float* __restrict__ out,
                                                         float* __restrict__ dg_part, int64_t P, int C, float eps,
                                                         const float* __restrict__ add_to, float* __restrict__ dx_amax,
                                                         _Float16* __restrict__ y_hi = nullptr, _Float16* __restrict__ y_lo = nullptr,
                                                         float* __restrict__ y_scale = nullptr) {
  constexpr int RPB = 256 / TPR;
  __shared__ float red[BWD ? 256 * VPL * 4 : 1];
  const int C4 = C >> 2;
  const int lane = threadIdx.x % TPR, rloc = threadIdx.x / TPR;
  float4 gv[VPL];
  bool cok[VPL];
#pragma unroll
  for (int v = 0; v < VPL; ++v) {
    int c4 = lane + v * TPR;
    cok[v] = c4 < C4;
    gv[v] = cok[v] ? reinterpret_cast<const float4*>(g)[c4] : make_float4(0, 0, 0, 0);
  }
  float dgacc[VPL][4];
#pragma unroll
  for (int v = 0; v < VPL; ++v)
#pragma unroll
    for (int j = 0; j < 4; ++j) dgacc[v][j] = 0.f;
  const float invC = 1.0f / (float)C;
  const int64_t rstride = (int64_t)gridDim.x * RPB;
  float ps = 1.0f;
  if (!BWD && y_hi && y_lo) {
    float mg = 0.f;
#pragma unroll
    for (int v = 0; v < VPL; ++v) mg = amax4(mg, gv[v]);
    ps = scale_from_amax(sqrtf((float)C) * group_max<TPR>(mg));
    if (blockIdx.x == 0 && threadIdx.x == 0) y_scale[0] = ps;
  }
  float am = 0.f;
  for (int64_t r0 = (int64_t)blockIdx.x * RPB; r0 < P; r0 += rstride) {
    int64_t r = r0 + rloc;
    bool rok = r < P;
    float4 xv[VPL];
    float s = 0.f;
#pragma unroll
    for (int v = 0; v < VPL; ++v) {
      xv[v] = (rok && cok[v]) ? reinterpret_cast<const float4*>(x + r * C)[lane + v * TPR] : make_float4(0, 0, 0, 0);
      s += (xv[v].x + xv[v].y) + (xv[v].z + xv[v].w);
    }
    float mean = group_sum<TPR>(s) * invC;
    float q = 0.f;
#pragma unroll
    for (int v = 0; v < VPL; ++v) {
      if (cok[v]) {
        xv[v].x -= mean; xv[v].y -= mean; xv[v].z -= mean; xv[v].w -= mean;
        q += (xv[v].x * xv[v].x + xv[v].y * xv[v].y) + (xv[v].z * xv[v].z + xv[v].w * xv[v].w);
      }
    }
    float var = group_sum<TPR>(q) * invC;
    float rstd = 1.0f / sqrtf(var + eps);
    if (!BWD) {
#pragma unroll
      for (int v = 0; v < VPL; ++v)
        if (rok && cok[v]) {
          float4 o;
          o.x = xv[v].x * rstd * gv[v].x; o.y = xv[v].y * rstd * gv[v].y;
          o.z = xv[v].z * rstd * gv[v].z; o.w = xv[v].w * rstd * gv[v].w;
          if (y_hi) {
            typedef _Float16 half4v __attribute__((ext_vector_type(4)));
            const float t[4] = {o.x, o.y, o.z, o.w};
            half4v h, l;
#pragma unroll
            for (int j = 0; j < 4; ++j) { _Float16 th, tl; plane_pack(t[j], ps, y_lo == nullptr, th, tl); h[j] = th; l[j] = tl; }
            reinterpret_cast<half4v*>(y_hi + r * C)[lane + v * TPR] = h;
            if (y_lo) reinterpret_cast<half4v*>(y_lo + r * C)[lane + v * TPR] = l;
            continue;
          }
          reinterpret_cast<float4*>(out + r * C)[lane + v * TPR] = o;
          am = amax4(am, o);
        }
    } else {
      float4 dv[VPL];
      float m1 = 0.f, m2 = 0.f;
#pragma unroll
      for (int v = 0; v < VPL; ++v) {
        dv[v] = (rok && cok[v]) ? reinterpret_cast<const float4*>(dy + r * C)[lane + v * TPR] : make_float4(0, 0, 0, 0);
        xv[v].x *= rstd; xv[v].y *= rstd; xv[v].z *= rstd; xv[v].w *= rstd;
        dgacc[v][0] += dv[v].x * xv[v].x; dgacc[v][1] += dv[v].y * xv[v].y;
        dgacc[v][2] += dv[v].z * xv[v].z; dgacc[v][3] += dv[v].w * xv[v].w;
        dv[v].x *= gv[v].x; dv[v].y *= gv[v].y; dv[v].z *= gv[v].z; dv[v].w *= gv[v].w;
        m1 += (dv[v].x + dv[v].y) + (dv[v].z + dv[v].w);
        m2 += (dv[v].x * xv[v].x + dv[v].y * xv[v].y) + (dv[v].z * xv[v].z + dv[v].w * xv[v].w);
      }
      m1 = group_sum<TPR>(m1) * invC;
      m2 = group_sum<TPR>(m2) * invC;
#pragma unroll
      for (int v = 0; v < VPL; ++v)
        if (rok && cok[v]) {
          float4 o;
          o.x = rstd * (dv[v].x - m1 - xv[v].x * m2); o.y = rstd * (dv[v].y - m1 - xv[v].y * m2);
          o.z = rstd * (dv[v].z - m1 - xv[v].z * m2); o.w = rstd * (dv[v].w - m1 - xv[v].w * m2);
          if (add_to) {
            const float4 t = reinterpret_cast<const float4*>(add_to + r * C)[lane + v * TPR];
            o.x += t.x; o.y += t.y; o.z += t.z; o.w += t.w;
          }
          reinterpret_cast<float4*>(out + r * C)[lane + v * TPR] = o;
          am = amax4(am, o);
        }
    }
  }
  if (!BWD && dg_part) amax_record_emit(am, dg_part, blockIdx.x);
  if (BWD && dx_amax) amax_record_emit(am, dx_amax, blockIdx.x);
  if (BWD) {
#pragma unroll
    for (int v = 0; v < VPL; ++v)
#pragma unroll
      for (int j = 0; j < 4; ++j) red[((rloc * TPR + lane) * VPL + v) * 4 + j] = dgacc[v][j];
    __syncthreads();
    if (rloc == 0) {
#pragma unroll
      for (int v = 0; v < VPL; ++v) {
        if (!cok[v]) continue;
        float a[4] = {0, 0, 0, 0};
        for (int t = 0; t < RPB; ++t)
#pragma unroll
          for (int j = 0; j < 4; ++j) a[j] += red[((t * TPR + lane) * VPL + v) * 4 + j];
        reinterpret_cast<float4*>(dg_part + (int64_t)blockIdx.x * C)[lane + v * TPR] = make_float4(a[0], a[1], a[2], a[3]);
      }
    }
  }
}

static inline int ln_blocks(int64_t P, int rpb) {
  int64_t nb = cdiv64(P, rpb);
  if (nb > 1024) nb = 1024;
  return (int)nb;
}
static inline void ln_shape(int C, int& tpr, int& vpl) {
  int c4 = C / 4;
  if (c4 <= 64) { tpr = pow2ceil(c4); if (tpr < 2) tpr = 2; vpl = 1; }
  else { tpr = 64; vpl = pow2ceil(cdiv(c4, 64)); }
}
template <bool BWD>
static int ln_launch(const float* x, const float* g, const float* dy, float* out, float* dgp, int64_t P, int C, float eps, hipStream_t st,
                     const float* add_to = nullptr, float* dx_amax = nullptr, _Float16* y_hi = nullptr, _Float16* y_lo = nullptr,
                     float* y_scale = nullptr) {
  int tpr, vpl;
  ln_shape(C, tpr, vpl);
  int nb = ln_blocks(P, 256 / tpr);
#define LN_CASE(T, V) layernorm_kernel<T, V, BWD><<<nb, 256, 0, st>>>(x, g, dy, out, dgp, P, C, eps, add_to, dx_amax, y_hi, y_lo, y_scale)
  if (vpl == 1) {
    switch (tpr) {
      case 2: LN_CASE(2, 1); break;
      case 4: LN_CASE(4, 1); break;
      case 8: LN_CASE(8, 1); break;
      case 16: LN_CASE(16, 1); break;
      case 32: LN_CASE(32, 1); break;
      default: LN_CASE(64, 1); break;
    }
  } else if (vpl == 2) LN_CASE(64, 2);
  else if (vpl == 4) LN_CASE(64, 4);
  else return WDNO_EUNSUPPORTED;
#undef LN_CASE
  return WDNO_OK;
}
extern "C" int wdno_layernorm_fwd_amax(const float* x, const float* g, float* y, float* amax_rec, int64_t P, int C, float eps,
                                       wdno_stream_t s) {
  WDNO_REQUIRE(P > 0 && C >= 4);
  if ((C & 3) || C > 1024) return WDNO_EUNSUPPORTED;
  int rc = ln_launch<false>(x, g, nullptr, y, amax_rec, P, C, eps, as_stream(s));
  if (rc) return rc;
  return wdno_check_launch();
}
extern "C" int wdno_layernorm_fwd_planes(const float* x, const float* g, void* y_hi, void* y_lo, float* y_scale, int64_t P, int C, float eps,
                                         wdno_stream_t s) {
  WDNO_REQUIRE(P > 0 && C >= 8);
  if ((C & 7) || C > 1024) return WDNO_EUNSUPPORTED;
  int rc = ln_launch<false>(x, g, nullptr, nullptr, nullptr, P, C, eps, as_stream(s), nullptr, nullptr, (_Float16*)y_hi, (_Float16*)y_lo, y_scale);
  if (rc) return rc;
  return wdno_check_launch();
}
extern "C" int wdno_layernorm_fwd(const float* x, const float* g, float* y, int64_t P, int C, float eps, wdno_stream_t s) {
  return wdno_layernorm_fwd_amax(x, g, y, nullptr, P, C, eps, s);
}
extern "C" size_t wdno_layernorm_bwd_ws_bytes(int64_t P, int C) { return (size_t)1024 * C * sizeof(float); }
extern "C" int wdno_layernorm_bwd_add_amax(const float* x, const float* g, const float* dy, const float* add_to, float* dx, float* dg,
                                           float* amax_rec, int64_t P, int C, float eps, void* ws, size_t ws_bytes, wdno_stream_t s) {
  WDNO_REQUIRE(P > 0 && C >= 4);
  if ((C & 3) || C > 1024) return WDNO_EUNSUPPORTED;
  if (ws_bytes < wdno_layernorm_bwd_ws_bytes(P, C)) return WDNO_EWORKSPACE;
  int tpr, vpl;
  ln_shape(C, tpr, vpl);
  int nb = ln_blocks(P, 256 / tpr);
  int rc = ln_launch<true>(x, g, dy, dx, (float*)ws, P, C, eps, as_stream(s), add_to, amax_rec);
  if (rc) return rc;
  partial_rows_sum_kernel<float><<<cdiv(C, 32), PRS_THREADS, 0, as_stream(s)>>>((const float*)ws, dg, nb, C);
  return wdno_check_launch();
}
extern "C" int wdno_layernorm_bwd_add(const float* x, const float* g, const float* dy, const float* add_to, float* dx, float* dg, int64_t P,
                                      int C, float eps, void* ws, size_t ws_bytes, wdno_stream_t s) {
  return wdno_layernorm_bwd_add_amax(x, g, dy, add_to, dx, dg, nullptr, P, C, eps, ws, ws_bytes, s);
}
extern "C" int wdno_layernorm_bwd(const float* x, const float* g, const float* dy, float* dx, float* dg, int64_t P, int C,
                                  float eps, void* ws, size_t ws_bytes, wdno_stream_t s) {
  return wdno_layernorm_bwd_add(x, g, dy, nullptr, dx, dg, P, C, eps, ws, ws_bytes, s);
}
```

wdno_amd/csrc/pointwise.hip:

```cpp
#include "common.h"

template <int ACT>
__device__ __forceinline__ float act_apply(float x) {
  if (ACT == 0) return silu_f(x);
  return 0.5f * x * (1.0f + erff(x * 0.70710678118654752440f));
}
template <int ACT>
__device__ __forceinline__ float act_grad(float x) {
  if (ACT == 0) return silu_grad_f(x);
  float cdf = 0.5f * (1.0f + erff(x * 0.70710678118654752440f));
  float pdf = 0.39894228040143267794f * expf(-0.5f * x * x);
  return cdf + x * pdf;
}

template <int ACT>
__global__ __launch_bounds__(256) void act_fwd_kernel(const float* __restrict__ x, float* __restrict__ y, int64_t n) {
  int64_t i = (int64_t)blockIdx.x * 256 + threadIdx.x;
  int64_t stride = (int64_t)gridDim.x * 256;
  int64_t n4 = n >> 2;
  for (int64_t k = i; k < n4; k += stride) {
    float4 v = reinterpret_cast<const float4*>(x)[k];
    v.x = act_apply<ACT>(v.x); v.y = act_apply<ACT>(v.y); v.z = act_apply<ACT>(v.z); v.w = act_apply<ACT>(v.w);
    reinterpret_cast<float4*>(y)[k] = v;
  }
  for (int64_t k = (n4 << 2) + i; k < n; k += stride) y[k] = act_apply<ACT>(x[k]);
}
template <int ACT>
__global__ __launch_bounds__(256) void act_bwd_kernel(const float* __restrict__ x, const float* __restrict__ dy,
                                                       float* __restrict__ dx, int64_t n) {
  int64_t i = (int64_t)blockIdx.x * 256 + threadIdx.x;
  int64_t stride = (int64_t)gridDim.x * 256;
  int64_t n4 = n >> 2;
  for (int64_t k = i; k < n4; k += stride) {
    float4 v = reinterpret_cast<const float4*>(x)[k];
    float4 g = reinterpret_cast<const float4*>(dy)[k];
    g.x *= act_grad<ACT>(v.x); g.y *= act_grad<ACT>(v.y); g.z *= act_grad<ACT>(v.z); g.w *= act_grad<ACT>(v.w);
    reinterpret_cast<float4*>(dx)[k] = g;
  }
  for (int64_t k = (n4 << 2) + i; k < n; k += stride) dx[k] = dy[k] * act_grad<ACT>(x[k]);
}

extern "C" int wdno_act_fwd(const float* x, float* y, int64_t n, int act, wdno_stream_t s) {
  WDNO_REQUIRE(n >= 0 && (act == 0 || act == 1));
  if (n == 0) return WDNO_OK;
  int grid = stream_grid(n / 4 + 1, 256);
  if (act == 0) act_fwd_kernel<0><<<grid, 256, 0, as_stream(s)>>>(x, y, n);
  else act_fwd_kernel<1><<<grid, 256, 0, as_stream(s)>>>(x, y, n);
  return wdno_check_launch();
}
extern "C" int wdno_act_bwd(const float* x, const float* dy, float* dx, int64_t n, int act, wdno_stream_t s) {
  WDNO_REQUIRE(n >= 0 && (act == 0 || act == 1));
  if (n == 0) return WDNO_OK;
  int grid = stream_grid(n / 4 + 1, 256);
  if (act == 0) act_bwd_kernel<0><<<grid, 256, 0, as_stream(s)>>>(x, dy, dx, n);
  else act_bwd_kernel<1><<<grid, 256, 0, as_stream(s)>>>(x, dy, dx, n);
  return wdno_check_launch();
}

__global__ __launch_bounds__(256) void add_kernel(const float* __restrict__ a, const float* __restrict__ b,
                                                   float* __restrict__ o, int64_t n, float* __restrict__ amax_rec) {
  int64_t i = (int64_t)blockIdx.x * 256 + threadIdx.x;
  int64_t stride = (int64_t)gridDim.x * 256;
  int64_t n4 = n >> 2;
  float am = 0.f;
  for (int64_t k = i; k < n4; k += stride) {
    float4 u = reinterpret_cast<const float4*>(a)[k];
    float4 v = reinterpret_cast<const float4*>(b)[k];
    u.x += v.x; u.y += v.y; u.z += v.z; u.w += v.w;
    reinterpret_cast<float4*>(o)[k] = u;
    am = amax4(am, u);
  }
  for (int64_t k = (n4 << 2) + i; k < n; k += stride) {
    float r = a[k] + b[k];
    o[k] = r;
    am = fmaxf(am, fabsf(r));
  }
  if (amax_rec) amax_record_emit(am, amax_rec, blockIdx.x);
}
extern "C" int wdno_add_amax(const float* a, const float* b, float* out, float* amax_rec, int64_t n, wdno_stream_t s) {
  WDNO_REQUIRE(n >= 0);
  if (n == 0) return WDNO_OK;
  add_kernel<<<stream_grid(n / 4 + 1, 256), 256, 0, as_stream(s)>>>(a, b, out, n, amax_rec);
  return wdno_check_launch();
}
extern "C" int wdno_add(const float* a, const float* b, float* out, int64_t n, wdno_stream_t s) {
  return wdno_add_amax(a, b, out, nullptr, n, s);
}

__global__ void sinusoidal_kernel(const int64_t* __restrict__ t, const float* __restrict__ freqs, float* __restrict__ out, int B, int dim) {
  int half = dim >> 1;
  int i = blockIdx.x * blockDim.x + threadIdx.x;
  if (i >= B * half) return;
  int b = i / half, k = i - b * half;
  float a = (float)t[b] * freqs[k];
  out[(int64_t)b * dim + k] = sinf(a);
  out[(int64_t)b * dim + half + k] = cosf(a);
}
extern "C" int wdno_sinusoidal_emb(const int64_t* t, const float* freqs, float* out, int B, int dim, wdno_stream_t s) {
  WDNO_REQUIRE(B > 0 && dim >= 4 && (dim % 2) == 0 && freqs != nullptr);
  int n = B * (dim / 2);
  sinusoidal_kernel<<<cdiv(n, 128), 128, 0, as_stream(s)>>>(t, freqs, out, B, dim);
  return wdno_check_launch();
}

__global__ __launch_bounds__(256) void nc_to_cl_kernel(const float* __restrict__ src, float* __restrict__ dst,
                                                        int C, int64_t S, int Cp) {
  __shared__ float tile[32][33];
  int64_t n = blockIdx.z;
  int64_t s0 = (int64_t)blockIdx.x * 32;
  int c0 = blockIdx.y * 32;
  int tx = threadIdx.x & 31, ty = threadIdx.x >> 5;
  const float* sp = src + n * (int64_t)C * S;
#pragma unroll
  for (int r = 0; r < 4; ++r) {
    int c = c0 + ty + r * 8;
    int64_t sidx = s0 + tx;
    tile[ty + r * 8][tx] = (c < C && sidx < S) ? sp[(int64_t)c * S + sidx] : 0.0f;
  }
  __syncthreads();
  float* dp = dst + n * S * (int64_t)Cp;
#pragma unroll
  for (int r = 0; r < 4; ++r) {
    int64_t sidx = s0 + ty + r * 8;
    int c = c0 + tx;
    if (sidx < S && c < Cp) dp[sidx * Cp + c] = tile[tx][ty + r * 8];
  }
}
__global__ __launch_bounds__(256) void cl_to_nc_kernel(const float* __restrict__ src, float* __restrict__ dst,
                                                        int C, int64_t S, int Cp) {
  __shared__ float tile[32][33];
  int64_t n = blockIdx.z;
  int64_t s0 = (int64_t)blockIdx.x * 32;
  int c0 = blockIdx.y * 32;
  int tx = threadIdx.x & 31, ty = threadIdx.x >> 5;
  const float* sp = src + n * S * (int64_t)Cp;
#pragma unroll
  for (int r = 0; r < 4; ++r) {
    int64_t sidx = s0 + ty + r * 8;
    int c = c0 + tx;
    tile[ty + r * 8][tx] = (sidx < S && c < C) ? sp[sidx * Cp + c] : 0.0f;
  }
  __syncthreads();
  float* dp = dst + n * (int64_t)C * S;
#pragma unroll
  for (int r = 0; r < 4; ++r) {
    int c = c0 + ty + r * 8;
    int64_t sidx = s0 + tx;
    if (c < C && sidx < S) dp[(int64_t)c * S + sidx] = tile[tx][ty + r * 8];
  }
}
extern "C" int wdno_nc_to_cl(const float* src, float* dst, int64_t N, int C, int64_t S, int Cp, wdno_stream_t s) {
  WDNO_REQUIRE(N > 0 && C > 0 && S > 0 && Cp >= C && N < 65536);
  dim3 grid((unsigned)cdiv64(S, 32), (unsigned)cdiv(Cp, 32), (unsigned)N);
  nc_to_cl_kernel<<<grid, 256, 0, as_stream(s)>>>(src, dst, C, S, Cp);
  return wdno_check_launch();
}
extern "C" int wdno_cl_to_nc(const float* src, float* dst, int64_t N, int C, int64_t S, int Cp, wdno_stream_t s) {
  WDNO_REQUIRE(N > 0 && C > 0 && S > 0 && Cp >= C && N < 65536);
  dim3 grid((unsigned)cdiv64(S, 32), (unsigned)cdiv(C, 32), (unsigned)N);
  cl_to_nc_kernel<<<grid, 256, 0, as_stream(s)>>>(src, dst, C, S, Cp);
  return wdno_check_launch();
}

__global__ __launch_bounds__(256) void concat2_kernel(const float4* __restrict__ a, int Ca4, const float4* __restrict__ b, int Cb4,
                                                       float4* __restrict__ out, int64_t total4, float* __restrict__ amax_rec) {
  int Ct4 = Ca4 + Cb4;
  int64_t stride = (int64_t)gridDim.x * 256;
  float am = 0.f;
  for (int64_t i = (int64_t)blockIdx.x * 256 + threadIdx.x; i < total4; i += stride) {
    int64_t p = i / Ct4;
    int c = (int)(i - p * Ct4);
    float4 v = (c < Ca4) ? a[p * Ca4 + c] : b[p * Cb4 + (c - Ca4)];
    out[i] = v;
    am = amax4(am, v);
  }
  if (amax_rec) amax_record_emit(am, amax_rec, blockIdx.x);
}
__global__ __launch_bounds__(256) void split2_kernel(const float4* __restrict__ in, float4* __restrict__ a, int Ca4,
                                                      float4* __restrict__ b, int Cb4, int64_t total4) {
  int Ct4 = Ca4 + Cb4;
  int64_t stride = (int64_t)gridDim.x * 256;
  for (int64_t i = (int64_t)blockIdx.x * 256 + threadIdx.x; i < total4; i += stride) {
    int64_t p = i / Ct4;
    int c = (int)(i - p * Ct4);
    float4 v = in[i];
    if (c < Ca4) a[p * Ca4 + c] = v; else b[p * Cb4 + (c - Ca4)] = v;
  }
}
extern "C" int wdno_concat2_cl_amax(const float* a, int Ca, const float* b, int Cb, float* out, float* amax_rec, int64_t P,
                                    wdno_stream_t s) {
  WDNO_REQUIRE(P > 0 && Ca > 0 && Cb > 0 && Ca % 4 == 0 && Cb % 4 == 0);
  int64_t total4 = P * ((Ca + Cb) / 4);
  concat2_kernel<<<stream_grid(total4, 256), 256, 0, as_stream(s)>>>((const float4*)a, Ca / 4, (const float4*)b, Cb / 4, (float4*)out,
                                                                     total4, amax_rec);
  return wdno_check_launch();
}
typedef _Float16 cc_half8 __attribute__((ext_vector_type(8)));
__global__ __launch_bounds__(256) void concat2_planes_kernel(const float* __restrict__ a, int Ca, const float* __restrict__ b, int Cb,
                                                              const float* __restrict__ rec_a, const float* __restrict__ rec_b,
                                                              _Float16* __restrict__ hi, _Float16* __restrict__ lo,
                                                              float* __restrict__ scale_out, int64_t P) {
  const bool single = lo == nullptr;
  const float s = single ? 1.0f : scale_from_amax(fmaxf(amax_record_read(rec_a), amax_record_read(rec_b)));
  if (!single && blockIdx.x == 0 && threadIdx.x == 0) scale_out[0] = s;
  const int Ct = Ca + Cb, g8 = Ct >> 3;
  const int64_t total = P * g8, stride = (int64_t)gridDim.x * 256;
  for (int64_t i = (int64_t)blockIdx.x * 256 + threadIdx.x; i < total; i += stride) {
    const int64_t p = i / g8;
    const int c0 = (int)(i - p * g8) * 8;
    const float* src = c0 < Ca ? a + p * Ca + c0 : b + p * Cb + (c0 - Ca);
    const float4 v0 = *reinterpret_cast<const float4*>(src), v1 = *reinterpret_cast<const float4*>(src + 4);
    const float v[8] = {v0.x, v0.y, v0.z, v0.w, v1.x, v1.y, v1.z, v1.w};
    cc_half8 h, l;
#pragma unroll
    for (int e = 0; e < 8; ++e) { _Float16 th, tl; plane_pack(v[e], s, single, th, tl); h[e] = th; l[e] = tl; }
    *reinterpret_cast<cc_half8*>(hi + p * Ct + c0) = h;
    if (!single) *reinterpret_cast<cc_half8*>(lo + p * Ct + c0) = l;
  }
}
extern "C" int wdno_concat2_cl_planes(const float* a, int Ca, const float* b, int Cb, const float* rec_a, const float* rec_b, void* hi,
                                      void* lo, float* scale_out, int64_t P, wdno_stream_t s) {
  WDNO_REQUIRE(P > 0 && Ca > 0 && Cb > 0 && Ca % 8 == 0 && Cb % 8 == 0 && hi != nullptr);
  WDNO_REQUIRE(lo == nullptr || (rec_a && rec_b && scale_out));
  const int64_t total = P * ((Ca + Cb) / 8);
  concat2_planes_kernel<<<stream_grid(total, 256), 256, 0, as_stream(s)>>>(a, Ca, b, Cb, rec_a, rec_b, (_Float16*)hi, (_Float16*)lo, scale_out, P);
  return wdno_check_launch();
}
extern "C" int wdno_concat2_cl(const float* a, int Ca, const float* b, int Cb, float* out, int64_t P, wdno_stream_t s) {
  return wdno_concat2_cl_amax(a, Ca, b, Cb, out, nullptr, P, s);
}
extern "C" int wdno_split2_cl(const float* in, float* a, int Ca, float* b, int Cb, int64_t P, wdno_stream_t s) {
  WDNO_REQUIRE(P > 0 && Ca > 0 && Cb > 0 && Ca % 4 == 0 && Cb % 4 == 0);
  int64_t total4 = P * ((Ca + Cb) / 4);
  split2_kernel<<<stream_grid(total4, 256), 256, 0, as_stream(s)>>>((const float4*)in, (float4*)a, Ca / 4, (float4*)b, Cb / 4, total4);
  return wdno_check_launch();
}

__global__ __launch_bounds__(256) void up2x_fwd_kernel(const float4* __restrict__ in, float4* __restrict__ out,
                                                        int H, int W, int C4, int64_t total4) {
  int64_t stride = (int64_t)gridDim.x * 256;
  int W2 = 2 * W, H2 = 2 * H;
  for (int64_t i = (int64_t)blockIdx.x * 256 + threadIdx.x; i < total4; i += stride) {
    int c = (int)(i % C4);
    int64_t p = i / C4;
    int w = (int)(p % W2);
    int64_t q = p / W2;
    int h = (int)(q % H2);
    int64_t n = q / H2;
    out[i] = in[((n * H + (h >> 1)) * W + (w >> 1)) * C4 + c];
  }
}
__global__ __launch_bounds__(256) void up2x_bwd_kernel(const float4* __restrict__ dout, float4* __restrict__ din,
                                                        int H, int W, int C4, int64_t total4) {
  int64_t stride = (int64_t)gridDim.x * 256;
  int W2 = 2 * W, H2 = 2 * H;
  for (int64_t i = (int64_t)blockIdx.x * 256 + threadIdx.x; i < total4; i += stride) {
    int c = (int)(i % C4);
    int64_t p = i / C4;
    int w = (int)(p % W);
    int64_t q = p / W;
    int h = (int)(q % H);
    int64_t n = q / H;
    int64_t base = ((n * H2 + 2 * h) * W2 + 2 * w) * C4 + c;
    float4 a = dout[base], b = dout[base + C4], d = dout[base + (int64_t)W2 * C4], e = dout[base + (int64_t)W2 * C4 + C4];
    float4 r;
    r.x = (a.x + b.x) + (d.x + e.x); r.y = (a.y + b.y) + (d.y + e.y);
    r.z = (a.z + b.z) + (d.z + e.z); r.w = (a.w + b.w) + (d.w + e.w);
    din[i] = r;
  }
}
extern "C" int wdno_upsample2x_cl_fwd(const float* in, float* out, int64_t N, int H, int W, int C, wdno_stream_t s) {
  WDNO_REQUIRE(N > 0 && H > 0 && W > 0 && C > 0 && C % 4 == 0);
  int64_t total4 = N * 4 * H * W * (C / 4);
  up2x_fwd_kernel<<<stream_grid(total4, 256), 256, 0, as_stream(s)>>>((const float4*)in, (float4*)out, H, W, C / 4, total4);
  return wdno_check_launch();
}
extern "C" int wdno_upsample2x_cl_bwd(const float* dout, float* din, int64_t N, int H, int W, int C, wdno_stream_t s) {
  WDNO_REQUIRE(N > 0 && H > 0 && W > 0 && C > 0 && C % 4 == 0);
  int64_t total4 = N * H * W * (C / 4);
  up2x_bwd_kernel<<<stream_grid(total4, 256), 256, 0, as_stream(s)>>>((const float4*)dout, (float4*)din, H, W, C / 4, total4);
  return wdno_check_launch();
}

__global__ __launch_bounds__(256) void upsample_coef_kernel(const float* __restrict__ in, float* __restrict__ out,
                                                             int a, int mid, int b, int c, int fa, int fb, int fc, int64_t total) {
  int64_t stride = (int64_t)gridDim.x * 256;
  int oc = c * fc, ob = b * fb, oa = a * fa;
  for (int64_t i = (int64_t)blockIdx.x * 256 + threadIdx.x; i < total; i += stride) {
    int ic = (int)(i % oc);
    int64_t r = i / oc;
    int ib = (int)(r % ob); r /= ob;
    int im = (int)(r % mid); r /= mid;
    int ia = (int)(r % oa);
    int64_t o = r / oa;
    out[i] = in[(((o * a + ia / fa) * mid + im) * b + ib / fb) * c + ic / fc];
  }
}
extern "C" int wdno_upsample_coef(const float* in, float* out, int64_t outer, int a, int mid, int b, int c,
                                  int fa, int fb, int fc, wdno_stream_t s) {
  WDNO_REQUIRE(outer > 0 && a > 0 && mid > 0 && b > 0 && c > 0 && fa > 0 && fb > 0 && fc > 0);
  int64_t total = outer * a * fa * mid * b * fb * c * fc;
  upsample_coef_kernel<<<stream_grid(total, 256), 256, 0, as_stream(s)>>>(in, out, a, mid, b, c, fa, fb, fc, total);
  return wdno_check_launch();
}

__global__ __launch_bounds__(256) void colsum_partial_kernel(const float* __restrict__ in, double* __restrict__ ws,
                                                              int64_t P, int C, int64_t rows_per_block) {
  __shared__ double red[4][64];
  int tx = threadIdx.x & 63, ty = threadIdx.x >> 6;
  int64_t r0 = (int64_t)blockIdx.x * rows_per_block;
  int64_t r1 = r0 + rows_per_block;
  if (r1 > P) r1 = P;
  for (int c0 = blockIdx.y * 64; c0 < C; c0 += 64 * gridDim.y) {
    int c = c0 + tx;
    double acc = 0.0;
    if (c < C)
      for (int64_t r = r0 + ty; r < r1; r += 4) acc += (double)in[r * C + c];
    red[ty][tx] = acc;
    __syncthreads();
    if (ty == 0 && c < C) ws[(int64_t)blockIdx.x * C + c] = (red[0][tx] + red[1][tx]) + (red[2][tx] + red[3][tx]);
    __syncthreads();
  }
}
static inline int colsum_blocks(int64_t P) {
  int64_t nb = cdiv64(P, 64);
  if (nb > 512) nb = 512;
  if (nb < 1) nb = 1;
  return (int)nb;
}
__global__ __launch_bounds__(256) void colsum_rows_kernel(const float* __restrict__ in, float* __restrict__ out, int P, int C) {
  const int c = blockIdx.x * 256 + threadIdx.x;
  if (c >= C) return;
  double a = 0.0;
  for (int p = 0; p < P; ++p) a += (double)in[(int64_t)p * C + c];
  out[c] = (float)a;
}
extern "C" size_t wdno_colsum_ws_bytes(int64_t P, int C) { return (size_t)colsum_blocks(P) * (size_t)C * sizeof(double); }
extern "C" int wdno_colsum(const float* in, float* out, int64_t P, int C, void* ws, size_t ws_bytes, wdno_stream_t s) {
  WDNO_REQUIRE(P > 0 && C > 0);
  if (P <= 64) {
    colsum_rows_kernel<<<cdiv(C, 256), 256, 0, as_stream(s)>>>(in, out, (int)P, C);
    return wdno_check_launch();
  }
  if (ws_bytes < wdno_colsum_ws_bytes(P, C)) return WDNO_EWORKSPACE;
  int nb = colsum_blocks(P);
  int64_t rpb = cdiv64(P, nb);
  int gy = cdiv(C, 64);
  if ((int64_t)gy * nb > 2048) gy = 2048 / nb > 1 ? 2048 / nb : 1;
  colsum_partial_kernel<<<dim3(nb, gy), 256, 0, as_stream(s)>>>(in, (double*)ws, P, C, rpb);
  partial_rows_sum_kernel<double><<<cdiv(C, 32), PRS_THREADS, 0, as_stream(s)>>>((const double*)ws, out, nb, C);
  return wdno_check_launch();
}

struct RowsSumArgs { wdno_rows_sum_item it[WDNO_ROWS_SUM_MAX]; int n; };
__global__ __launch_bounds__(PRS_THREADS) void rows_sum_multi_kernel(RowsSumArgs a) {
  int b = (int)blockIdx.x, i = 0;
  for (; i < a.n; ++i) {
    const int nb = (a.it[i].ncols + 31) >> 5;
    if (b < nb) break;
    b -= nb;
  }
  if (i >= a.n) return;
  const wdno_rows_sum_item& t = a.it[i];
  if (t.is_double) partial_rows_sum_body<double>((const double*)t.part + t.col0, t.out, t.rows, t.ncols, b, t.stride);
  else partial_rows_sum_body<float>((const float*)t.part + t.col0, t.out, t.rows, t.ncols, b, t.stride);
}
extern "C" int wdno_rows_sum_multi(const wdno_rows_sum_item* items, int n_items, wdno_stream_t s) {
  WDNO_REQUIRE(n_items >= 0 && (items || n_items == 0));
  for (int base = 0; base < n_items; base += WDNO_ROWS_SUM_MAX) {
    RowsSumArgs a;
    a.n = n_items - base < WDNO_ROWS_SUM_MAX ? n_items - base : WDNO_ROWS_SUM_MAX;
    int blocks = 0;
    for (int i = 0; i < a.n; ++i) {
      a.it[i] = items[base + i];
      WDNO_REQUIRE(a.it[i].part && a.it[i].out && a.it[i].rows > 0 && a.it[i].ncols > 0 && a.it[i].col0 >= 0 && a.it[i].stride >= a.it[i].col0 + a.it[i].ncols);
      blocks += cdiv(a.it[i].ncols, 32);
    }
    rows_sum_multi_kernel<<<blocks, PRS_THREADS, 0, as_stream(s)>>>(a);
  }
  return wdno_check_launch();
}

__global__ __launch_bounds__(256) void sumsq_partial_kernel(const float* __restrict__ g, int64_t n, double* __restrict__ ws) {
  __shared__ double red[4];
  int64_t stride = (int64_t)gridDim.x * 256;
  int64_t n4 = n >> 2;
  double acc = 0.0;
  for (int64_t k = (int64_t)blockIdx.x * 256 + threadIdx.x; k < n4; k += stride) {
    float4 v = reinterpret_cast<const float4*>(g)[k];
    acc += (double)v.x * v.x + (double)v.y * v.y + (double)v.z * v.z + (double)v.w * v.w;
  }
  for (int64_t k = (n4 << 2) + (int64_t)blockIdx.x * 256 + threadIdx.x; k < n; k += stride) acc += (double)g[k] * g[k];
  acc = wave_sum_d(acc);
  if ((threadIdx.x & 63) == 0) red[threadIdx.x >> 6] = acc;
  __syncthreads();
  if (threadIdx.x == 0) ws[blockIdx.x] = (red[0] + red[1]) + (red[2] + red[3]);
}
__global__ __launch_bounds__(256) void sum_final_kernel(const double* __restrict__ ws, int nb, float* __restrict__ out, float scale) {
  __shared__ double red[4];
  double acc = 0.0;
  for (int i = threadIdx.x; i < nb; i += 256) acc += ws[i];
  acc = wave_sum_d(acc);
  if ((threadIdx.x & 63) == 0) red[threadIdx.x >> 6] = acc;
  __syncthreads();
  if (threadIdx.x == 0) out[0] = (float)(((red[0] + red[1]) + (red[2] + red[3])) * (double)scale);
}
extern "C" size_t wdno_sumsq_ws_bytes(int64_t n) { return (size_t)stream_grid(n / 4 + 1, 256) * sizeof(double); }
extern "C" int wdno_sumsq(const float* g, int64_t n, float* out, void* ws, size_t ws_bytes, wdno_stream_t s) {
  WDNO_REQUIRE(n > 0);
  if (ws_bytes < wdno_sumsq_ws_bytes(n)) return WDNO_EWORKSPACE;
  int nb = stream_grid(n / 4 + 1, 256);
  sumsq_partial_kernel<<<nb, 256, 0, as_stream(s)>>>(g, n, (double*)ws);
  sum_final_kernel<<<1, 256, 0, as_stream(s)>>>((const double*)ws, nb, out, 1.0f);
  return wdno_check_launch();
}

__global__ __launch_bounds__(256) void adam_kernel(float* __restrict__ p, const float* __restrict__ g, float* __restrict__ m,
                                                    float* __restrict__ v, int64_t n, const float* __restrict__ sumsq,
                                                    float max_norm, float grad_scale, float step_size, float beta1, float beta2,
                                                    float eps, float bc2_sqrt) {
  float coef = grad_scale;
  if (sumsq != nullptr && max_norm > 0.0f) {
    float total = sqrtf(sumsq[0]) * grad_scale;
    float c = max_norm / (total + 1e-6f);
    coef *= fminf(c, 1.0f);
  }
  int64_t stride = (int64_t)gridDim.x * 256;
  for (int64_t k = (int64_t)blockIdx.x * 256 + threadIdx.x; k < n; k += stride) {
    float gr = g[k] * coef;
    float mk = m[k] + (gr - m[k]) * (1.0f - beta1);
    float vk = v[k] * beta2 + (1.0f - beta2) * gr * gr;
    m[k] = mk;
    v[k] = vk;
    float denom = sqrtf(vk) / bc2_sqrt + eps;
    p[k] = p[k] - step_size * (mk / denom);
  }
}
extern "C" int wdno_adam_clip_step(float* p, const float* g, float* m, float* v, int64_t n, const float* sumsq, float max_norm,
                                   float grad_scale, float lr, float beta1, float beta2, float eps, int step, wdno_stream_t s) {
  WDNO_REQUIRE(n > 0 && step >= 1);
  double bc1 = 1.0 - pow((double)beta1, (double)step);
  double bc2 = 1.0 - pow((double)beta2, (double)step);
  float step_size = (float)((double)lr / bc1);
  float bc2_sqrt = (float)sqrt(bc2);
  adam_kernel<<<stream_grid(n, 256), 256, 0, as_stream(s)>>>(p, g, m, v, n, sumsq, max_norm, grad_scale, step_size, beta1, beta2, eps, bc2_sqrt);
  return wdno_check_launch();
}

__global__ __launch_bounds__(256) void ema_kernel(float* __restrict__ e, const float* __restrict__ p, int64_t n, float w) {
  int64_t stride = (int64_t)gridDim.x * 256;
  for (int64_t k = (int64_t)blockIdx.x * 256 + threadIdx.x; k < n; k += stride) e[k] = e[k] + (p[k] - e[k]) * w;
}
extern "C" int wdno_ema_update(float* ema, const float* p, int64_t n, float beta, wdno_stream_t s) {
  WDNO_REQUIRE(n > 0);
  ema_kernel<<<stream_grid(n, 256), 256, 0, as_stream(s)>>>(ema, p, n, 1.0f - beta);
  return wdno_check_launch();
}

__global__ __launch_bounds__(256) void gather_items_kernel(const wdno_copy_item* __restrict__ tab) {
  const wdno_copy_item it = tab[blockIdx.y];
  const float* __restrict__ src = (const float*)it.src;
  float* __restrict__ dst = (float*)it.dst;
  const int64_t n = it.n;
  if (src == dst || (int64_t)blockIdx.x * 256 >= n) return;
  const int64_t stride = (int64_t)gridDim.x * 256;
  for (int64_t i0 = (int64_t)blockIdx.x * 256 + threadIdx.x; i0 < n; i0 += 4 * stride) {
    float v[4];
#pragma unroll
    for (int u = 0; u < 4; ++u) {
      const int64_t i = i0 + u * stride;
      v[u] = (src && i < n) ? src[i] : 0.f;
    }
#pragma unroll
    for (int u = 0; u < 4; ++u) {
      const int64_t i = i0 + u * stride;
      if (i < n) dst[i] = v[u];
    }
  }
}
extern "C" int wdno_gather_items(const void* table, int n_items, int blocks_per_item, wdno_stream_t s) {
  WDNO_REQUIRE(table && n_items > 0 && n_items <= 65535 && blocks_per_item > 0);
  gather_items_kernel<<<dim3((unsigned)blocks_per_item, (unsigned)n_items), 256, 0, as_stream(s)>>>((const wdno_copy_item*)table);
  return wdno_check_launch();
}

__global__ __launch_bounds__(256) void relpos_fwd_kernel(const float* __restrict__ w, const int64_t* __restrict__ bucket, float* __restrict__ out,
                                                          int nn, int heads) {
  for (int e = threadIdx.x; e < heads * nn; e += 256) {
    const int h = e / nn, ij = e - h * nn;
    out[e] = w[bucket[ij] * heads + h];
  }
}
template <bool STAGED>
__global__ __launch_bounds__(256) void relpos_bwd_kernel(const float* __restrict__ dbias, const int64_t* __restrict__ bucket, float* __restrict__ dw,
                                                          int nn, int heads, int nb) {
  extern __shared__ float sm[];
  int* sb = (int*)(sm + (size_t)heads * nn);
  if (STAGED) {
    for (int e = threadIdx.x; e < heads * nn; e += 256) sm[e] = dbias[e];
    for (int e = threadIdx.x; e < nn; e += 256) sb[e] = (int)bucket[e];
    __syncthreads();
  }
  for (int o = threadIdx.x; o < nb * heads; o += 256) {
    const int bk = o / heads, h = o - bk * heads;
    float acc = 0.f;
    for (int ij = 0; ij < nn; ++ij) {
      const int bb = STAGED ? sb[ij] : (int)bucket[ij];
      const float v = STAGED ? sm[h * nn + ij] : dbias[(size_t)h * nn + ij];
      if (bb == bk) acc += v;
    }
    dw[o] = acc;
  }
}
extern "C" int wdno_relpos_bias_fwd(const float* w, const int64_t* bucket, float* out, int n, int heads, wdno_stream_t s) {
  WDNO_REQUIRE(n > 0 && heads > 0);
  relpos_fwd_kernel<<<1, 256, 0, as_stream(s)>>>(w, bucket, out, n * n, heads);
  return wdno_check_launch();
}
extern "C" int wdno_relpos_bias_bwd(const float* dbias, const int64_t* bucket, float* dw, int n, int heads, int num_buckets, wdno_stream_t s) {
  WDNO_REQUIRE(n > 0 && heads > 0 && num_buckets > 0 && num_buckets * heads <= 8192);
  const size_t lds = (size_t)n * n * (heads + 1) * sizeof(float);
  if (lds <= 48 * 1024) relpos_bwd_kernel<true><<<1, 256, lds, as_stream(s)>>>(dbias, bucket, dw, n * n, heads, num_buckets);
  else relpos_bwd_kernel<false><<<1, 256, 0, as_stream(s)>>>(dbias, bucket, dw, n * n, heads, num_buckets);
  return wdno_check_launch();
}
```

Measured before the change: 32.68.

## Vectorize SiLU with fast reciprocal division and templatize groupnorm kernels on flags

Replaces the IEEE division in SiLU and its gradient with an rcp-plus-Newton sequence, taken only when every lane's input is in a safe range, and evaluates several values together to expose ILP. Groupnorm partial, apply and backward kernels are now templated on the SILU, SINGLE and GSHARED flags, which removes runtime branches. The apply-planes and backward-partial kernels also process multiple rows per iteration to keep more loads in flight. Debug kernels are added to count bitwise mismatches between the fast and reference SiLU, and the pointwise activation path keeps the reference version.

```diff
diff --git a/include/wdno_hip.h b/include/wdno_hip.h
--- a/include/wdno_hip.h
+++ b/include/wdno_hip.h
@@ -273,6 +273,8 @@
 
 int wdno_act_fwd(const float* x, float* y, int64_t n, int act, wdno_stream_t s);
 int wdno_act_bwd(const float* x, const float* dy, float* dx, int64_t n, int act, wdno_stream_t s);
+int wdno_debug_silu_mismatches(uint64_t n0, uint64_t n1, uint64_t* out_counts, wdno_stream_t s);
+int wdno_debug_silu_ref(const float* z, float* y, int64_t n, int grad, wdno_stream_t s);
 int wdno_add(const float* a, const float* b, float* out, int64_t n, wdno_stream_t s);
 int wdno_add_amax(const float* a, const float* b, float* out, float* amax_rec, int64_t n, wdno_stream_t s);
 int wdno_sinusoidal_emb(const int64_t* t, const float* freqs, float* out, int B, int dim, wdno_stream_t s);
diff --git a/wdno_amd/_lib.py b/wdno_amd/_lib.py
--- a/wdno_amd/_lib.py
+++ b/wdno_amd/_lib.py
@@ -170,6 +170,8 @@
     'wdno_linattn_bwd_planes': (I, [P, P, P, P, P, P, P, P, P, P, P, Z, L, I, I, F, P]),
     'wdno_act_fwd': (I, [P, P, L, I, P]),
     'wdno_act_bwd': (I, [P, P, P, L, I, P]),
+    'wdno_debug_silu_mismatches': (I, [C.c_uint64, C.c_uint64, P, P]),
+    'wdno_debug_silu_ref': (I, [P, P, L, I, P]),
     'wdno_linear_rows_fwd': (I, [P, I, P, I, P, P, I, I, I, I, P]),
     'wdno_linear_rows_wgrad': (I, [P, I, P, I, P, P, I, I, I, P]),
     'wdno_linear_multi_fwd': (I, [P, I, I, P, P, I, I, P]),
diff --git a/wdno_amd/csrc/common.h b/wdno_amd/csrc/common.h
--- a/wdno_amd/csrc/common.h
+++ b/wdno_amd/csrc/common.h
@@ -136,9 +136,50 @@
   partial_rows_sum_body<T>(part, out, nb, C, (int)blockIdx.x);
 }
 
-__device__ __forceinline__ float silu_f(float z) { return z / (1.0f + expf(-z)); }
-__device__ __forceinline__ float silu_grad_f(float z) {
+__device__ __forceinline__ float silu_f_ref(float z) { return z / (1.0f + expf(-z)); }
+__device__ __forceinline__ float silu_grad_f_ref(float z) {
   float sg = 1.0f / (1.0f + expf(-z));
   return sg * (1.0f + z * (1.0f - sg));
 }
+__device__ __forceinline__ float div_unscaled_f(float n, float d) {
+  float r = __builtin_amdgcn_rcpf(d);
+  r = __builtin_fmaf(__builtin_fmaf(-d, r, 1.0f), r, r);
+  float q = n * r;
+  q = __builtin_fmaf(__builtin_fmaf(-d, q, n), r, q);
+  return __builtin_fmaf(__builtin_fmaf(-d, q, n), r, q);
+}
+__device__ __forceinline__ bool silu_fast_ok(float z) { const float a = fabsf(z); return a >= 0x1p-60f && a < 80.0f; }
+__device__ __forceinline__ bool silu_grad_fast_ok(float z) { return fabsf(z) < 80.0f; }
+template <int NV>
+__device__ __forceinline__ void silu_v(float (&z)[NV]) {
+  float d[NV];
+  bool ok = true;
+#pragma unroll
+  for (int j = 0; j < NV; ++j) { d[j] = 1.0f + expf(-z[j]); ok = ok && silu_fast_ok(z[j]); }
+  if (__builtin_expect(ok, 1)) {
+#pragma unroll
+    for (int j = 0; j < NV; ++j) z[j] = div_unscaled_f(z[j], d[j]);
+  } else {
+#pragma unroll
+    for (int j = 0; j < NV; ++j) z[j] = z[j] / d[j];
+  }
+}
+template <int NV>
+__device__ __forceinline__ void silu_grad_v(float (&z)[NV]) {
+  float d[NV];
+  bool ok = true;
+#pragma unroll
+  for (int j = 0; j < NV; ++j) { d[j] = 1.0f + expf(-z[j]); ok = ok && silu_grad_fast_ok(z[j]); }
+  if (__builtin_expect(ok, 1)) {
+#pragma unroll
+    for (int j = 0; j < NV; ++j) d[j] = div_unscaled_f(1.0f, d[j]);
+  } else {
+#pragma unroll
+    for (int j = 0; j < NV; ++j) d[j] = 1.0f / d[j];
+  }
+#pragma unroll
+  for (int j = 0; j < NV; ++j) z[j] = d[j] * (1.0f + z[j] * (1.0f - d[j]));
+}
+__device__ __forceinline__ float silu_f(float z) { float v[1] = {z}; silu_v<1>(v); return v[0]; }
+__device__ __forceinline__ float silu_grad_f(float z) { float v[1] = {z}; silu_grad_v<1>(v); return v[0]; }
 #endif
diff --git a/wdno_amd/csrc/norm.hip b/wdno_amd/csrc/norm.hip
--- a/wdno_amd/csrc/norm.hip
+++ b/wdno_amd/csrc/norm.hip
@@ -2,6 +2,28 @@
 #include <type_traits>
 
 #define GN_MAXC 1024
+#ifndef GN_ROWS_IN_FLIGHT
+#define GN_ROWS_IN_FLIGHT 2
+#endif
+#ifndef GN_CHAINS
+#define GN_CHAINS 8
+#endif
+#ifndef GN_PARTIAL_ROWS
+#define GN_PARTIAL_ROWS 2
+#endif
+#ifndef GN_WAVES_FWD
+#define GN_WAVES_FWD 1
+#endif
+#ifndef GN_WAVES_BWD
+#define GN_WAVES_BWD 1
+#endif
+template <bool GRAD> __device__ __forceinline__ void gn_silu8(float* v) {
+#pragma unroll
+  for (int k = 0; k < 8; k += GN_CHAINS) {
+    if (GRAD) silu_grad_v(*reinterpret_cast<float(*)[GN_CHAINS]>(v + k));
+    else silu_v(*reinterpret_cast<float(*)[GN_CHAINS]>(v + k));
+  }
+}
 
 struct gn_bf16 {};
 template <typename T> struct gn_ld;
@@ -14,7 +36,7 @@
     return make_float4(__uint_as_float(u.x << 16), __uint_as_float(u.x & 0xffff0000u), __uint_as_float(u.y << 16), __uint_as_float(u.y & 0xffff0000u));
   }
 };
-template <typename T> __device__ __forceinline__ void gn_ld8(const void* p, int64_t e, float (&v)[8]) {
+template <typename T> __device__ __forceinline__ void gn_ld8(const void* p, int64_t e, float* v) {
   const float4 a = gn_ld<T>::ld4(p, e), b = gn_ld<T>::ld4(p, e + 4);
   v[0] = a.x; v[1] = a.y; v[2] = a.z; v[3] = a.w; v[4] = b.x; v[5] = b.y; v[6] = b.z; v[7] = b.w;
 }
@@ -32,11 +54,11 @@
   return (int)c;
 }
 
-template <int MODE, typename XT = float, typename DT = float>
-__global__ __launch_bounds__(256) void gn_partial_kernel(const void* __restrict__ x, const void* __restrict__ dy,
+template <int MODE, typename XT = float, typename DT = float, bool SILU = false>
+__global__ __launch_bounds__(256, GN_WAVES_BWD) void gn_partial_kernel(const void* __restrict__ x, const void* __restrict__ dy,
                                                           const float* __restrict__ cb , const float* __restrict__ gb ,
                                                           double* __restrict__ part, int64_t S, int C, int cg, int G, int txp,
-                                                          int64_t rows_per_chunk, int silu, float* __restrict__ mx = nullptr) {
+                                                          int64_t rows_per_chunk, float* __restrict__ mx = nullptr) {
   __shared__ double red[256 * 8];
   __shared__ float redm[8];
   float m0[4] = {0.f, 0.f, 0.f, 0.f}, m1[4] = {0.f, 0.f, 0.f, 0.f};
@@ -62,6 +84,46 @@
     }
     const int64_t e0 = ((int64_t)n * S) * C + tx * 4;
     constexpr int RIF = std::is_same<XT, gn_bf16>::value ? 8 : 4;
+    auto rows = [&](auto nr, const float4* vv, const float4* dd, int u0) {
+      constexpr int NR = decltype(nr)::value;
+      if (MODE == 0) {
+#pragma unroll
+        for (int u = 0; u < NR; ++u) {
+          const float4 v = vv[u0 + u];
+          const float xv[4] = {v.x, v.y, v.z, v.w};
+#pragma unroll
+          for (int j = 0; j < 4; ++j) {
+            s0[j] += (double)xv[j]; s1[j] = __builtin_fma((double)xv[j], (double)xv[j], s1[j]); m0[j] = fmaxf(m0[j], fabsf(xv[j]));
+          }
+        }
+      } else {
+        float g[NR * 4];
+        if (SILU) {
+#pragma unroll
+          for (int u = 0; u < NR; ++u) {
+            const float4 v = vv[u0 + u];
+            const float xv[4] = {v.x, v.y, v.z, v.w};
+#pragma unroll
+            for (int j = 0; j < 4; ++j) g[u * 4 + j] = ca[j] * xv[j] + cbb[j];
+          }
+          silu_grad_v(g);
+        }
+#pragma unroll
+        for (int u = 0; u < NR; ++u) {
+          const float4 v = vv[u0 + u], d = dd[u0 + u];
+          const float xv[4] = {v.x, v.y, v.z, v.w}, dv[4] = {d.x, d.y, d.z, d.w};
+#pragma unroll
+          for (int j = 0; j < 4; ++j) {
+            float dz = dv[j];
+            if (SILU) dz *= g[u * 4 + j];
+            float xh = (xv[j] - mean[j]) * rstd[j];
+            s0[j] += (double)dz;
+            s1[j] = __builtin_fma((double)dz, (double)xh, s1[j]);
+            m0[j] = fmaxf(m0[j], fabsf(dz)); m1[j] = fmaxf(m1[j], fabsf(xh));
+          }
+        }
+      }
+    };
     for (int64_t rb = r0 + ty; rb < r1; rb += RIF * nty) {
       float4 vv[RIF], dd[RIF];
 #pragma unroll
@@ -71,26 +133,14 @@
         vv[u] = ok ? gn_ld<XT>::ld4(x, e0 + r * C) : make_float4(0.f, 0.f, 0.f, 0.f);
         if (MODE == 1) dd[u] = ok ? gn_ld<DT>::ld4(dy, e0 + r * C) : make_float4(0.f, 0.f, 0.f, 0.f);
       }
-#pragma unroll
-      for (int u = 0; u < RIF; ++u) {
-        if (rb + u * nty >= r1) break;
-        const float4 v = vv[u];
-        float xv[4] = {v.x, v.y, v.z, v.w};
-        if (MODE == 0) {
-#pragma unroll
-          for (int j = 0; j < 4; ++j) { s0[j] += (double)xv[j]; s1[j] += (double)xv[j] * (double)xv[j]; m0[j] = fmaxf(m0[j], fabsf(xv[j])); }
-        } else {
-          const float4 d = dd[u];
-          float dv[4] = {d.x, d.y, d.z, d.w};
-#pragma unroll
-          for (int j = 0; j < 4; ++j) {
-            float dz = dv[j];
-            if (silu) dz *= silu_grad_f(ca[j] * xv[j] + cbb[j]);
-            float xh = (xv[j] - mean[j]) * rstd[j];
-            s0[j] += (double)dz;
-            s1[j] += (double)dz * (double)xh;
-            m0[j] = fmaxf(m0[j], fabsf(dz)); m1[j] = fmaxf(m1[j], fabsf(xh));
-          }
+      if (MODE == 1 && rb + (RIF - 1) * nty < r1) {
+#pragma unroll
+        for (int u = 0; u < RIF; u += GN_PARTIAL_ROWS) rows(std::integral_constant<int, GN_PARTIAL_ROWS>(), vv, dd, u);
+      } else {
+#pragma unroll
+        for (int u = 0; u < RIF; ++u) {
+          if (rb + u * nty >= r1) break;
+          rows(std::integral_constant<int, 1>(), vv, dd, u);
         }
       }
     }
@@ -247,9 +297,9 @@
   }
 }
 
-template <typename XT = float>
+template <typename XT, bool SILU>
 __global__ __launch_bounds__(256) void gn_apply_kernel(const void* __restrict__ x, const float* __restrict__ cb, float* __restrict__ y,
-                                                        int64_t S, int C, int silu, float* __restrict__ amax_rec) {
+                                                        int64_t S, int C, float* __restrict__ amax_rec) {
   const int n = blockIdx.y;
   const int C4 = C >> 2;
   const int64_t total4 = S * C4;
@@ -262,9 +312,9 @@
     int c4 = (int)(i % C4);
     float4 v = gn_ld<XT>::ld4(x, xe + i * 4);
     float4 k0 = cbp[c4 * 4 + 0], k1 = cbp[c4 * 4 + 1], k2 = cbp[c4 * 4 + 2], k3 = cbp[c4 * 4 + 3];
-    float4 o;
-    o.x = k0.x * v.x + k0.y; o.y = k1.x * v.y + k1.y; o.z = k2.x * v.z + k2.y; o.w = k3.x * v.w + k3.y;
-    if (silu) { o.x = silu_f(o.x); o.y = silu_f(o.y); o.z = silu_f(o.z); o.w = silu_f(o.w); }
+    float z[4] = {k0.x * v.x + k0.y, k1.x * v.y + k1.y, k2.x * v.z + k2.y, k3.x * v.w + k3.y};
+    if (SILU) silu_v(z);
+    const float4 o = make_float4(z[0], z[1], z[2], z[3]);
     yp[i] = o;
     am = amax4(am, o);
   }
@@ -351,9 +401,10 @@
   }
 }
 
+template <bool SILU>
 __global__ __launch_bounds__(256) void gn_bwd_apply_kernel(const float* __restrict__ x, const float* __restrict__ dy,
                                                             const float* __restrict__ cb, const float* __restrict__ gb,
-                                                            float* __restrict__ dx, int64_t S, int C, int cg, int G, int silu,
+                                                            float* __restrict__ dx, int64_t S, int C, int cg, int G,
                                                             float* __restrict__ amax_rec) {
   const int n = blockIdx.y;
   const int C4 = C >> 2;
@@ -368,16 +419,22 @@
   for (int64_t i = (int64_t)blockIdx.x * 256 + threadIdx.x; i < total4; i += stride) {
     int c4 = (int)(i % C4);
     float4 v = xp[i], d = dp[i];
-    float xv[4] = {v.x, v.y, v.z, v.w}, dv[4] = {d.x, d.y, d.z, d.w}, o[4];
+    float xv[4] = {v.x, v.y, v.z, v.w}, dv[4] = {d.x, d.y, d.z, d.w}, o[4], g[4];
+    float4 k[4], gq[4];
 #pragma unroll
     for (int j = 0; j < 4; ++j) {
       int c = c4 * 4 + j;
-      float4 k = cbp[c];
-      float4 gq = gbp[c / cg];
+      k[j] = cbp[c];
+      gq[j] = gbp[c / cg];
+      g[j] = k[j].x * xv[j] + k[j].y;
+    }
+    if (SILU) silu_grad_v(g);
+#pragma unroll
+    for (int j = 0; j < 4; ++j) {
       float dz = dv[j];
-      if (silu) dz *= silu_grad_f(k.x * xv[j] + k.y);
-      float xh = (xv[j] - gq.x) * gq.y;
-      o[j] = k.z * dz - gq.z - xh * gq.w;
+      if (SILU) dz *= g[j];
+      float xh = (xv[j] - gq[j].x) * gq[j].y;
+      o[j] = k[j].z * dz - gq[j].z - xh * gq[j].w;
     }
     op[i] = make_float4(o[0], o[1], o[2], o[3]);
     am = fmaxf(fmaxf(am, fmaxf(fabsf(o[0]), fabsf(o[1]))), fmaxf(fabsf(o[2]), fabsf(o[3])));
@@ -386,62 +443,76 @@
 }
 
 typedef _Float16 gn_half8 __attribute__((ext_vector_type(8)));
-template <typename XT = float>
-__global__ __launch_bounds__(256) void gn_apply_planes_kernel(const void* __restrict__ x, const float* __restrict__ cb,
-                                                               _Float16* __restrict__ hi, _Float16* __restrict__ lo,
-                                                               float* __restrict__ scale_out, const float* __restrict__ rec,
-                                                               int64_t S, int C, int silu) {
+#define GN_ROWS(i0)                                                                         \
+  do {                                                                                      \
+    int64_t i = (i0);                                                                       \
+    if (GN_ROWS_IN_FLIGHT == 2)                                                             \
+      for (; i + stride < total8; i += 2 * stride) rows(std::integral_constant<int, 2>(), i); \
+    else                                                                                    \
+      for (; i + stride < total8; i += stride) rows(std::integral_constant<int, 1>(), i);   \
+    if (i < total8) rows(std::integral_constant<int, 1>(), i);                              \
+  } while (0)
+template <typename XT, bool SILU, bool SINGLE>
+__global__ __launch_bounds__(256, GN_WAVES_FWD) void gn_apply_planes_kernel(const void* __restrict__ x, const float* __restrict__ cb,
+                                                                  _Float16* __restrict__ hi, _Float16* __restrict__ lo,
+                                                                  float* __restrict__ scale_out, const float* __restrict__ rec,
+                                                                  int64_t S, int C) {
   const int n = blockIdx.y;
   const int C8 = C >> 3;
   const int64_t total8 = S * C8;
-  const bool single = lo == nullptr;
-  const float s = single ? 1.0f : scale_from_amax(amax_record_read(rec));
-  if (!single && blockIdx.x == 0 && blockIdx.y == 0 && threadIdx.x == 0) scale_out[0] = s;
+  const float s = SINGLE ? 1.0f : scale_from_amax(amax_record_read(rec));
+  if (!SINGLE && blockIdx.x == 0 && blockIdx.y == 0 && threadIdx.x == 0) scale_out[0] = s;
   const int64_t xe = (int64_t)n * S * C;
   _Float16* hp = hi + (int64_t)n * S * C;
-  _Float16* lp = single ? nullptr : lo + (int64_t)n * S * C;
+  _Float16* lp = SINGLE ? nullptr : lo + (int64_t)n * S * C;
   const float4* cbp = reinterpret_cast<const float4*>(cb + (int64_t)n * C * 4);
   const int64_t stride = (int64_t)gridDim.x * 256;
   const int c0 = (int)(((int64_t)blockIdx.x * 256 + threadIdx.x) % C8) * 8;
   float ka[8], kb[8];
 #pragma unroll
   for (int j = 0; j < 8; ++j) { const float4 k = cbp[c0 + j]; ka[j] = k.x; kb[j] = k.y; }
-  for (int64_t i = (int64_t)blockIdx.x * 256 + threadIdx.x; i < total8; i += stride) {
-    float xv[8];
-    gn_ld8<XT>(x, xe + i * 8, xv);
-    gn_half8 h, l;
-#pragma unroll
-    for (int j = 0; j < 8; ++j) {
-      float o = ka[j] * xv[j] + kb[j];
-      if (silu) o = silu_f(o);
-      _Float16 th, tl;
-      plane_pack(o, s, single, th, tl);
-      h[j] = th; l[j] = tl;
-    }
-    *reinterpret_cast<gn_half8*>(hp + i * 8) = h;
-    if (!single) *reinterpret_cast<gn_half8*>(lp + i * 8) = l;
-  }
-}
-
-template <typename XT = float>
-__global__ __launch_bounds__(256) void gn_apply_add_planes_kernel(const void* __restrict__ x, const float* __restrict__ cb,
-                                                                   const float* __restrict__ res, float* __restrict__ y,
-                                                                   _Float16* __restrict__ hi, _Float16* __restrict__ lo,
-                                                                   float* __restrict__ scale_out, const float* __restrict__ rec,
-                                                                   const float* __restrict__ rec_res, float* __restrict__ amax_out,
-                                                                   int64_t S, int C, int silu) {
+  auto rows = [&](auto nr, int64_t i) {
+    constexpr int NR = decltype(nr)::value;
+    float z[NR * 8];
+#pragma unroll
+    for (int r = 0; r < NR; ++r) gn_ld8<XT>(x, xe + (i + r * stride) * 8, z + r * 8);
+#pragma unroll
+    for (int r = 0; r < NR; ++r) {
+      float o[8];
+#pragma unroll
+      for (int j = 0; j < 8; ++j) o[j] = ka[j] * z[r * 8 + j] + kb[j];
+      if (SILU) gn_silu8<false>(o);
+      gn_half8 h, l;
+#pragma unroll
+      for (int j = 0; j < 8; ++j) {
+        _Float16 th, tl;
+        plane_pack(o[j], s, SINGLE, th, tl);
+        h[j] = th; l[j] = tl;
+      }
+      *reinterpret_cast<gn_half8*>(hp + (i + r * stride) * 8) = h;
+      if (!SINGLE) *reinterpret_cast<gn_half8*>(lp + (i + r * stride) * 8) = l;
+    }
+  };
+  GN_ROWS((int64_t)blockIdx.x * 256 + threadIdx.x);
+}
+
+template <typename XT, bool SILU, bool PLANES, bool SINGLE>
+__global__ __launch_bounds__(256, GN_WAVES_FWD) void gn_apply_add_planes_kernel(const void* __restrict__ x, const float* __restrict__ cb,
+                                                                      const float* __restrict__ res, float* __restrict__ y,
+                                                                      _Float16* __restrict__ hi, _Float16* __restrict__ lo,
+                                                                      float* __restrict__ scale_out, const float* __restrict__ rec,
+                                                                      const float* __restrict__ rec_res, float* __restrict__ amax_out,
+                                                                      int64_t S, int C) {
   const int n = blockIdx.y;
   const int C8 = C >> 3;
   const int64_t total8 = S * C8;
-  const bool planes = hi != nullptr;
-  const bool single = lo == nullptr;
-  const float s = single ? 1.0f : scale_from_amax(amax_record_read(rec) + amax_record_read(rec_res));
-  if (!single && blockIdx.x == 0 && blockIdx.y == 0 && threadIdx.x == 0) scale_out[0] = s;
+  const float s = SINGLE ? 1.0f : scale_from_amax(amax_record_read(rec) + amax_record_read(rec_res));
+  if (!SINGLE && blockIdx.x == 0 && blockIdx.y == 0 && threadIdx.x == 0) scale_out[0] = s;
   const int64_t xe = (int64_t)n * S * C;
   const float* rp = res + (int64_t)n * S * C;
   float* yp = y + (int64_t)n * S * C;
-  _Float16* hp = planes ? hi + (int64_t)n * S * C : nullptr;
-  _Float16* lp = single ? nullptr : lo + (int64_t)n * S * C;
+  _Float16* hp = PLANES ? hi + (int64_t)n * S * C : nullptr;
+  _Float16* lp = SINGLE ? nullptr : lo + (int64_t)n * S * C;
   const float4* cbp = reinterpret_cast<const float4*>(cb + (int64_t)n * C * 4);
   const int64_t stride = (int64_t)gridDim.x * 256;
   const int c0 = (int)(((int64_t)blockIdx.x * 256 + threadIdx.x) % C8) * 8;
@@ -449,75 +520,102 @@
 #pragma unroll
   for (int j = 0; j < 8; ++j) { const float4 k = cbp[c0 + j]; ka[j] = k.x; kb[j] = k.y; }
   float am = 0.f;
-  for (int64_t i = (int64_t)blockIdx.x * 256 + threadIdx.x; i < total8; i += stride) {
-    float xv[8];
-    gn_ld8<XT>(x, xe + i * 8, xv);
-    const float4 r0 = *reinterpret_cast<const float4*>(rp + i * 8), r1 = *reinterpret_cast<const float4*>(rp + i * 8 + 4);
-    const float rv[8] = {r0.x, r0.y, r0.z, r0.w, r1.x, r1.y, r1.z, r1.w};
-    float ov[8];
-    gn_half8 h, l;
-#pragma unroll
-    for (int j = 0; j < 8; ++j) {
-      float o = ka[j] * xv[j] + kb[j];
-      if (silu) o = silu_f(o);
-      o += rv[j];
-      ov[j] = o;
-      am = fmaxf(am, fabsf(o));
-      _Float16 th, tl;
-      plane_pack(o, s, single, th, tl);
-      h[j] = th; l[j] = tl;
-    }
-    *reinterpret_cast<float4*>(yp + i * 8) = make_float4(ov[0], ov[1], ov[2], ov[3]);
-    *reinterpret_cast<float4*>(yp + i * 8 + 4) = make_float4(ov[4], ov[5], ov[6], ov[7]);
-    if (planes) *reinterpret_cast<gn_half8*>(hp + i * 8) = h;
-    if (planes && !single) *reinterpret_cast<gn_half8*>(lp + i * 8) = l;
-  }
+  auto rows = [&](auto nr, int64_t i) {
+    constexpr int NR = decltype(nr)::value;
+    float z[NR * 8], rv[NR * 8];
+#pragma unroll
+    for (int r = 0; r < NR; ++r) {
+      gn_ld8<XT>(x, xe + (i + r * stride) * 8, z + r * 8);
+      gn_ld8<float>(rp, (i + r * stride) * 8, rv + r * 8);
+    }
+#pragma unroll
+    for (int r = 0; r < NR; ++r) {
+      float ov[8];
+#pragma unroll
+      for (int j = 0; j < 8; ++j) ov[j] = ka[j] * z[r * 8 + j] + kb[j];
+      if (SILU) gn_silu8<false>(ov);
+      gn_half8 h, l;
+#pragma unroll
+      for (int j = 0; j < 8; ++j) {
+        const float o = ov[j] + rv[r * 8 + j];
+        ov[j] = o;
+        am = fmaxf(am, fabsf(o));
+        _Float16 th, tl;
+        plane_pack(o, s, SINGLE, th, tl);
+        h[j] = th; l[j] = tl;
+      }
+      *reinterpret_cast<float4*>(yp + (i + r * stride) * 8) = make_float4(ov[0], ov[1], ov[2], ov[3]);
+      *reinterpret_cast<float4*>(yp + (i + r * stride) * 8 + 4) = make_float4(ov[4], ov[5], ov[6], ov[7]);
+      if (PLANES) *reinterpret_cast<gn_half8*>(hp + (i + r * stride) * 8) = h;
+      if (PLANES && !SINGLE) *reinterpret_cast<gn_half8*>(lp + (i + r * stride) * 8) = l;
+    }
+  };
+  GN_ROWS((int64_t)blockIdx.x * 256 + threadIdx.x);
   if (amax_out) amax_record_emit(am, amax_out, blockIdx.y * gridDim.x + blockIdx.x);
 }
 
-template <typename XT = float, typename DT = float>
-__global__ __launch_bounds__(256) void gn_bwd_apply_planes_kernel(const void* __restrict__ x, const void* __restrict__ dy,
+template <typename XT, typename DT, bool SILU, bool SINGLE, bool GSHARED>
+__global__ __launch_bounds__(256, GN_WAVES_BWD) void gn_bwd_apply_planes_kernel(const void* __restrict__ x, const void* __restrict__ dy,
                                                                    const float* __restrict__ cb, const float* __restrict__ gb,
                                                                    _Float16* __restrict__ hi, _Float16* __restrict__ lo,
                                                                    float* __restrict__ scale_out, const float* __restrict__ rec,
-                                                                   double* __restrict__ csp, int64_t S, int C, int cg, int G, int silu) {
+                                                                   double* __restrict__ csp, int64_t S, int C, int cg, int G) {
   __shared__ double red[256][9];
   const int n = blockIdx.y;
   const int C8 = C >> 3;
   const int64_t total8 = S * C8;
-  const bool single = lo == nullptr;
-  const float s = single ? 1.0f : scale_from_amax(amax_record_read(rec));
-  if (!single && blockIdx.x == 0 && blockIdx.y == 0 && threadIdx.x == 0) scale_out[0] = s;
+  const float s = SINGLE ? 1.0f : scale_from_amax(amax_record_read(rec));
+  if (!SINGLE && blockIdx.x == 0 && blockIdx.y == 0 && threadIdx.x == 0) scale_out[0] = s;
   const int64_t xe = (int64_t)n * S * C;
   _Float16* hp = hi + (int64_t)n * S * C;
-  _Float16* lp = single ? nullptr : lo + (int64_t)n * S * C;
+  _Float16* lp = SINGLE ? nullptr : lo + (int64_t)n * S * C;
   const float4* cbp = reinterpret_cast<const float4*>(cb + (int64_t)n * C * 4);
   const float4* gbp = reinterpret_cast<const float4*>(gb + (int64_t)n * G * 4);
   const int64_t stride = (int64_t)gridDim.x * 256;
   const int c0 = (int)(((int64_t)blockIdx.x * 256 + threadIdx.x) % C8) * 8;
-  float4 kk[8], gq[8];
-#pragma unroll
-  for (int j = 0; j < 8; ++j) { kk[j] = cbp[c0 + j]; gq[j] = gbp[(c0 + j) / cg]; }
+  float ka[8], kb[8], kz[8];
+  float4 gq[GSHARED ? 1 : 8];
+#pragma unroll
+  for (int j = 0; j < 8; ++j) {
+    const float4 k = cbp[c0 + j];
+    ka[j] = k.x; kb[j] = k.y; kz[j] = k.z;
+    if (!GSHARED || j == 0) gq[GSHARED ? 0 : j] = gbp[(c0 + j) / cg];
+  }
   double acc[8] = {0, 0, 0, 0, 0, 0, 0, 0};
-  for (int64_t i = (int64_t)blockIdx.x * 256 + threadIdx.x; i < total8; i += stride) {
-    float xv[8], dv[8];
-    gn_ld8<XT>(x, xe + i * 8, xv);
-    gn_ld8<DT>(dy, xe + i * 8, dv);
-    gn_half8 h, l;
-#pragma unroll
-    for (int j = 0; j < 8; ++j) {
-      float dz = dv[j];
-      if (silu) dz *= silu_grad_f(kk[j].x * xv[j] + kk[j].y);
-      const float xh = (xv[j] - gq[j].x) * gq[j].y;
-      const float o = kk[j].z * dz - gq[j].z - xh * gq[j].w;
-      acc[j] += (double)o;
-      _Float16 th, tl;
-      plane_pack(o, s, single, th, tl);
-      h[j] = th; l[j] = tl;
-    }
-    *reinterpret_cast<gn_half8*>(hp + i * 8) = h;
-    if (!single) *reinterpret_cast<gn_half8*>(lp + i * 8) = l;
-  }
+  auto rows = [&](auto nr, int64_t i) {
+    constexpr int NR = decltype(nr)::value;
+    float xv[NR * 8], dv[NR * 8];
+#pragma unroll
+    for (int r = 0; r < NR; ++r) {
+      gn_ld8<XT>(x, xe + (i + r * stride) * 8, xv + r * 8);
+      gn_ld8<DT>(dy, xe + (i + r * stride) * 8, dv + r * 8);
+    }
+#pragma unroll
+    for (int r = 0; r < NR; ++r) {
+      float g[8];
+      if (SILU) {
+#pragma unroll
+        for (int j = 0; j < 8; ++j) g[j] = ka[j] * xv[r * 8 + j] + kb[j];
+        gn_silu8<true>(g);
+      }
+      gn_half8 h, l;
+#pragma unroll
+      for (int j = 0; j < 8; ++j) {
+        float dz = dv[r * 8 + j];
+        if (SILU) dz *= g[j];
+        const float4 q = gq[GSHARED ? 0 : j];
+        const float xh = (xv[r * 8 + j] - q.x) * q.y;
+        const float o = kz[j] * dz - q.z - xh * q.w;
+        acc[j] += (double)o;
+        _Float16 th, tl;
+        plane_pack(o, s, SINGLE, th, tl);
+        h[j] = th; l[j] = tl;
+      }
+      *reinterpret_cast<gn_half8*>(hp + (i + r * stride) * 8) = h;
+      if (!SINGLE) *reinterpret_cast<gn_half8*>(lp + (i + r * stride) * 8) = l;
+    }
+  };
+  GN_ROWS((int64_t)blockIdx.x * 256 + threadIdx.x);
 #pragma unroll
   for (int j = 0; j < 8; ++j) red[threadIdx.x][j] = acc[j];
   __syncthreads();
@@ -544,6 +642,7 @@
   if ((C & 3) || C > GN_MAXC || (C % G) != 0) return WDNO_EUNSUPPORTED;
   return WDNO_OK;
 }
+#define GN_FLAG(cond, NAME, ...) do { if (cond) { constexpr bool NAME = true; __VA_ARGS__; } else { constexpr bool NAME = false; __VA_ARGS__; } } while (0)
 #define GN_PARTIAL0(XB, ...) do { if (XB) gn_partial_kernel<0, gn_bf16><<<__VA_ARGS__; else gn_partial_kernel<0, float><<<__VA_ARGS__; } while (0)
 extern "C" int wdno_groupnorm_act_fwd_amax_t(const void* x, int x_bf16, const float* gamma, const float* beta, const float* ss, float* y,
                                       float* stats, float* amax_rec, int64_t N, int64_t S, int C, int G, float eps, int silu,
@@ -558,12 +657,13 @@
   const int txp = pow2ceil(C / 4);
   const int64_t rpc = cdiv64(S, nchunk);
   hipStream_t st = as_stream(s);
-  GN_PARTIAL0(x_bf16, dim3(nchunk, (unsigned)N), 256, 0, st>>>(x, nullptr, nullptr, nullptr, part, S, C, C / G, G, txp, rpc, 0));
+  GN_PARTIAL0(x_bf16, dim3(nchunk, (unsigned)N), 256, 0, st>>>(x, nullptr, nullptr, nullptr, part, S, C, C / G, G, txp, rpc));
   gn_finalize_kernel<<<dim3((unsigned)N, gn_slices(C, G)), 256, 0, st>>>(part, nullptr, gamma, beta, ss, stats, cb, gb, S, C, G, nchunk, eps);
   int gx = stream_grid(S * (C / 4), 256);
   if (gx > 512) gx = 512;
-  if (x_bf16) gn_apply_kernel<gn_bf16><<<dim3(gx, (unsigned)N), 256, 0, st>>>(x, cb, y, S, C, silu, amax_rec);
-  else gn_apply_kernel<float><<<dim3(gx, (unsigned)N), 256, 0, st>>>(x, cb, y, S, C, silu, amax_rec);
+  GN_FLAG(silu, SILU,
+          if (x_bf16) gn_apply_kernel<gn_bf16, SILU><<<dim3(gx, (unsigned)N), 256, 0, st>>>(x, cb, y, S, C, amax_rec);
+          else gn_apply_kernel<float, SILU><<<dim3(gx, (unsigned)N), 256, 0, st>>>(x, cb, y, S, C, amax_rec));
   return wdno_check_launch();
 }
 extern "C" int wdno_groupnorm_act_fwd_amax(const float* x, const float* gamma, const float* beta, const float* ss, float* y,
@@ -589,11 +689,11 @@
   const int txp = pow2ceil(C / 4);
   const int64_t rpc = cdiv64(S, nchunk);
   hipStream_t st = as_stream(s);
-  gn_partial_kernel<1><<<dim3(nchunk, (unsigned)N), 256, 0, st>>>(x, dy, cb, gb, part, S, C, C / G, G, txp, rpc, silu);
+  GN_FLAG(silu, SILU, gn_partial_kernel<1, float, float, SILU><<<dim3(nchunk, (unsigned)N), 256, 0, st>>>(x, dy, cb, gb, part, S, C, C / G, G, txp, rpc));
   gn_bwd_finalize_kernel<<<dim3((unsigned)N, gn_slices(C, G)), 256, 0, st>>>(part, gamma, beta, ss, gb, dgb_partial, dss, S, C, G, nchunk);
   int gx = stream_grid(S * (C / 4), 256);
   if (gx > 512) gx = 512;
-  gn_bwd_apply_kernel<<<dim3(gx, (unsigned)N), 256, 0, st>>>(x, dy, cb, gb, dx, S, C, C / G, G, silu, amax_rec);
+  GN_FLAG(silu, SILU, gn_bwd_apply_kernel<SILU><<<dim3(gx, (unsigned)N), 256, 0, st>>>(x, dy, cb, gb, dx, S, C, C / G, G, amax_rec));
   return wdno_check_launch();
 }
 extern "C" int wdno_groupnorm_act_bwd(const float* x, const float* dy, const float* gamma, const float* beta, const float* ss,
@@ -622,12 +722,13 @@
   const int txp = pow2ceil(C / 4);
   const int64_t rpc = cdiv64(S, nchunk);
   hipStream_t st = as_stream(s);
-  GN_PARTIAL0(x_bf16, dim3(nchunk, (unsigned)N), 256, 0, st>>>(x, nullptr, nullptr, nullptr, part, S, C, C / G, G, txp, rpc, 0, y_lo ? mx : nullptr));
+  GN_PARTIAL0(x_bf16, dim3(nchunk, (unsigned)N), 256, 0, st>>>(x, nullptr, nullptr, nullptr, part, S, C, C / G, G, txp, rpc, y_lo ? mx : nullptr));
   gn_finalize_kernel<<<dim3((unsigned)N, gn_slices(C, G)), 256, 0, st>>>(part, nullptr, gamma, beta, ss, stats, cb, gb, S, C, G, nchunk, eps, mx, y_lo ? bound_rec : nullptr);
   int gx = stream_grid(S * (C / 8), 256);
   if (gx > 512) gx = 512;
-  if (x_bf16) gn_apply_planes_kernel<gn_bf16><<<dim3(gx, (unsigned)N), 256, 0, st>>>(x, cb, (_Float16*)y_hi, (_Float16*)y_lo, y_scale, bound_rec, S, C, silu);
-  else gn_apply_planes_kernel<float><<<dim3(gx, (unsigned)N), 256, 0, st>>>(x, cb, (_Float16*)y_hi, (_Float16*)y_lo, y_scale, bound_rec, S, C, silu);
+  GN_FLAG(silu, SILU, GN_FLAG(y_lo == nullptr, SINGLE,
+          if (x_bf16) gn_apply_planes_kernel<gn_bf16, SILU, SINGLE><<<dim3(gx, (unsigned)N), 256, 0, st>>>(x, cb, (_Float16*)y_hi, (_Float16*)y_lo, y_scale, bound_rec, S, C);
+          else gn_apply_planes_kernel<float, SILU, SINGLE><<<dim3(gx, (unsigned)N), 256, 0, st>>>(x, cb, (_Float16*)y_hi, (_Float16*)y_lo, y_scale, bound_rec, S, C)));
   return wdno_check_launch();
 }
 extern "C" int wdno_groupnorm_act_fwd_planes(const float* x, const float* gamma, const float* beta, const float* ss, void* y_hi, void* y_lo,
@@ -654,14 +755,16 @@
   const int txp = pow2ceil(C / 4);
   const int64_t rpc = cdiv64(S, nchunk);
   hipStream_t st = as_stream(s);
-  GN_PARTIAL0(x_bf16, dim3(nchunk, (unsigned)N), 256, 0, st>>>(x, nullptr, nullptr, nullptr, part, S, C, C / G, G, txp, rpc, 0, y_lo ? mx : nullptr));
+  GN_PARTIAL0(x_bf16, dim3(nchunk, (unsigned)N), 256, 0, st>>>(x, nullptr, nullptr, nullptr, part, S, C, C / G, G, txp, rpc, y_lo ? mx : nullptr));
   gn_finalize_kernel<<<dim3((unsigned)N, gn_slices(C, G)), 256, 0, st>>>(part, nullptr, gamma, beta, ss, stats, cb, gb, S, C, G, nchunk, eps, mx, y_lo ? bound_rec : nullptr);
   int gx = stream_grid(S * (C / 8), 256);
   if (gx > 512) gx = 512;
-  if (x_bf16) gn_apply_add_planes_kernel<gn_bf16><<<dim3(gx, (unsigned)N), 256, 0, st>>>(x, cb, residual, y, (_Float16*)y_hi, (_Float16*)y_lo, y_scale, bound_rec,
-                                                                                       res_rec, y_amax_rec, S, C, silu);
-  else gn_apply_add_planes_kernel<float><<<dim3(gx, (unsigned)N), 256, 0, st>>>(x, cb, residual, y, (_Float16*)y_hi, (_Float16*)y_lo, y_scale, bound_rec, res_rec,
-                                                                           y_amax_rec, S, C, silu);
+#define GN_K_APPLY_ADD(XT, PLANES, SINGLE) gn_apply_add_planes_kernel<XT, SILU, PLANES, SINGLE><<<dim3(gx, (unsigned)N), 256, 0, st>>>( \
+    x, cb, residual, y, (_Float16*)y_hi, (_Float16*)y_lo, y_scale, bound_rec, res_rec, y_amax_rec, S, C)
+  GN_FLAG(silu, SILU,
+          if (x_bf16) { if (!y_hi) GN_K_APPLY_ADD(gn_bf16, false, true); else if (!y_lo) GN_K_APPLY_ADD(gn_bf16, true, true); else GN_K_APPLY_ADD(gn_bf16, true, false); }
+          else { if (!y_hi) GN_K_APPLY_ADD(float, false, true); else if (!y_lo) GN_K_APPLY_ADD(float, true, true); else GN_K_APPLY_ADD(float, true, false); });
+#undef GN_K_APPLY_ADD
   return wdno_check_launch();
 }
 extern "C" int wdno_groupnorm_act_add_fwd_planes(const float* x, const float* gamma, const float* beta, const float* ss, const float* residual,
@@ -722,12 +825,13 @@
 #define GN_BWD_TYPES(KERNEL, ...) do { \
     if (x_bf16 && dy_bf16) KERNEL(gn_bf16, gn_bf16, __VA_ARGS__); else if (x_bf16) KERNEL(gn_bf16, float, __VA_ARGS__); \
     else if (dy_bf16) KERNEL(float, gn_bf16, __VA_ARGS__); else KERNEL(float, float, __VA_ARGS__); } while (0)
-#define GN_K_PARTIAL1(XT, DT, ...) gn_partial_kernel<1, XT, DT><<<dim3(nchunk, (unsigned)N), 256, 0, st>>>(__VA_ARGS__)
-#define GN_K_BWD_APPLY(XT, DT, ...) gn_bwd_apply_planes_kernel<XT, DT><<<dim3(gx, (unsigned)N), 256, 0, st>>>(__VA_ARGS__)
-  GN_BWD_TYPES(GN_K_PARTIAL1, x, dy, cb, gb, part, S, C, C / G, G, txp, rpc, silu, dx_lo ? mx : nullptr);
+#define GN_K_PARTIAL1(XT, DT, ...) gn_partial_kernel<1, XT, DT, SILU><<<dim3(nchunk, (unsigned)N), 256, 0, st>>>(__VA_ARGS__)
+#define GN_K_BWD_APPLY(XT, DT, ...) gn_bwd_apply_planes_kernel<XT, DT, SILU, SINGLE, GSHARED><<<dim3(gx, (unsigned)N), 256, 0, st>>>(__VA_ARGS__)
+  GN_FLAG(silu, SILU, GN_BWD_TYPES(GN_K_PARTIAL1, x, dy, cb, gb, part, S, C, C / G, G, txp, rpc, dx_lo ? mx : nullptr));
   gn_bwd_finalize_kernel<<<dim3((unsigned)N, gn_slices(C, G)), 256, 0, st>>>(part, gamma, beta, ss, gb, dgb_partial, dss, S, C, G, nchunk, cb, mx, dx_lo ? bound_rec : nullptr);
   const int gx = gn_planes_grid(N, S, C);
-  GN_BWD_TYPES(GN_K_BWD_APPLY, x, dy, cb, gb, (_Float16*)dx_hi, (_Float16*)dx_lo, dx_scale, bound_rec, csp, S, C, C / G, G, silu);
+  GN_FLAG(silu, SILU, GN_FLAG(dx_lo == nullptr, SINGLE, GN_FLAG((C / G) % 8 == 0, GSHARED,
+          GN_BWD_TYPES(GN_K_BWD_APPLY, x, dy, cb, gb, (_Float16*)dx_hi, (_Float16*)dx_lo, dx_scale, bound_rec, csp, S, C, C / G, G))));
   const int nbx = dx_colsum ? cdiv(C, 32) : 0, nby = dgb_sum ? cdiv(2 * C, 32) : 0;
   if (nbx + nby) gn_bwd_tail_kernel<<<nbx + nby, PRS_THREADS, 0, st>>>(csp, dx_colsum, (int)N * gx, C, nbx, dgb_partial, dgb_sum, (int)N);
   return wdno_check_launch();
diff --git a/wdno_amd/csrc/pointwise.hip b/wdno_amd/csrc/pointwise.hip
--- a/wdno_amd/csrc/pointwise.hip
+++ b/wdno_amd/csrc/pointwise.hip
@@ -2,12 +2,12 @@
 
 template <int ACT>
 __device__ __forceinline__ float act_apply(float x) {
-  if (ACT == 0) return silu_f(x);
+  if (ACT == 0) return silu_f_ref(x);
   return 0.5f * x * (1.0f + erff(x * 0.70710678118654752440f));
 }
 template <int ACT>
 __device__ __forceinline__ float act_grad(float x) {
-  if (ACT == 0) return silu_grad_f(x);
+  if (ACT == 0) return silu_grad_f_ref(x);
   float cdf = 0.5f * (1.0f + erff(x * 0.70710678118654752440f));
   float pdf = 0.39894228040143267794f * expf(-0.5f * x * x);
   return cdf + x * pdf;
@@ -524,3 +524,35 @@
   else relpos_bwd_kernel<false><<<1, 256, 0, as_stream(s)>>>(dbias, bucket, dw, n * n, heads, num_buckets);
   return wdno_check_launch();
 }
+
+__global__ __launch_bounds__(256) void silu_mismatch_kernel(uint64_t n0, uint64_t n1, unsigned long long* __restrict__ counts) {
+  const uint64_t stride = (uint64_t)gridDim.x * 256;
+  unsigned c0 = 0, c1 = 0;
+  for (uint64_t p = n0 + (uint64_t)blockIdx.x * 256 + threadIdx.x; p < n1; p += stride) {
+    const float z = __uint_as_float((unsigned)p);
+    c0 += __float_as_uint(silu_f(z)) != __float_as_uint(silu_f_ref(z));
+    c1 += __float_as_uint(silu_grad_f(z)) != __float_as_uint(silu_grad_f_ref(z));
+  }
+#pragma unroll
+  for (int o = 32; o > 0; o >>= 1) { c0 += __shfl_xor(c0, o, 64); c1 += __shfl_xor(c1, o, 64); }
+  if ((threadIdx.x & 63) == 0) {
+    if (c0) atomicAdd(counts, (unsigned long long)c0);
+    if (c1) atomicAdd(counts + 1, (unsigned long long)c1);
+  }
+}
+__global__ __launch_bounds__(256) void silu_ref_kernel(const float* __restrict__ z, float* __restrict__ y, int64_t n, int grad) {
+  const int64_t stride = (int64_t)gridDim.x * 256;
+  for (int64_t k = (int64_t)blockIdx.x * 256 + threadIdx.x; k < n; k += stride) y[k] = grad ? silu_grad_f_ref(z[k]) : silu_f_ref(z[k]);
+}
+extern "C" int wdno_debug_silu_mismatches(uint64_t n0, uint64_t n1, uint64_t* out_counts, wdno_stream_t s) {
+  WDNO_REQUIRE(out_counts && n0 <= n1 && n1 <= ((uint64_t)1 << 32));
+  if (n0 == n1) return WDNO_OK;
+  silu_mismatch_kernel<<<stream_grid((int64_t)(n1 - n0), 256), 256, 0, as_stream(s)>>>(n0, n1, reinterpret_cast<unsigned long long*>(out_counts));
+  return wdno_check_launch();
+}
+extern "C" int wdno_debug_silu_ref(const float* z, float* y, int64_t n, int grad, wdno_stream_t s) {
+  WDNO_REQUIRE(n >= 0 && (n == 0 || (z && y)));
+  if (n == 0) return WDNO_OK;
+  silu_ref_kernel<<<stream_grid(n, 256), 256, 0, as_stream(s)>>>(z, y, n, grad);
+  return wdno_check_launch();
+}
```

Result: no change. 32.79 (median of 6 runs) (+0.3%).
